# jhbastek/PhysicsInformedDiffusionModels

Measured on NVIDIA H100. Metric: train samples/s Darcy 64x64 PIDM, higher is better.
Workload: dtype bf16

## Files before the change

physicsinformeddiffusionmodels_b200/csrc/attention_fused.cu:

```cuda
#include "common.cuh"
#include "mma_util.cuh"
#include "pidm.h"

namespace pidm {

constexpr int LF_C = 32;

__device__ __forceinline__ uint32_t movm_t(uint32_t x) {
    uint32_t y;
    asm volatile("movmatrix.sync.aligned.m8n8.trans.b16 %0, %1;" : "=r"(y) : "r"(x));
    return y;
}

__device__ __forceinline__ void load_w_frags(uint32_t (&w)[2][4][2], const __nv_bfloat16* __restrict__ Wrows, int lane) {
    const int g = lane >> 2, t = lane & 3;
#pragma unroll
    for (int ks = 0; ks < 2; ++ks)
#pragma unroll
        for (int nt = 0; nt < 4; ++nt) {
            const uint32_t* row = reinterpret_cast<const uint32_t*>(Wrows + (size_t)(nt * 8 + g) * LF_C + ks * 16 + 2 * t);
            w[ks][nt][0] = __ldg(row);
            w[ks][nt][1] = __ldg(row + 4);
        }
}
template <int MT>
__device__ __forceinline__ void load_x_frags(uint32_t (&a)[MT][2][4], const __nv_bfloat16* Xs, int lane) {
#pragma unroll
    for (int mt = 0; mt < MT; ++mt)
#pragma unroll
        for (int ks = 0; ks < 2; ++ks) frag_a_rowmajor(a[mt][ks], Xs, LW_PITCH, mt * 16, ks * 16, lane);
}
template <int MT>
__device__ __forceinline__ void project(float (&c)[MT][4][4], const uint32_t (&a)[MT][2][4], const uint32_t (&w)[2][4][2]) {
#pragma unroll
    for (int mt = 0; mt < MT; ++mt)
#pragma unroll
        for (int nt = 0; nt < 4; ++nt) {
#pragma unroll
            for (int i = 0; i < 4; ++i) c[mt][nt][i] = 0.f;
#pragma unroll
            for (int ks = 0; ks < 2; ++ks) mma_bf16(c[mt][nt], a[mt][ks], w[ks][nt][0], w[ks][nt][1]);
        }
}
__device__ __forceinline__ void frag_softmax(float (&c)[4][4], float mul) {
#pragma unroll
    for (int half = 0; half < 2; ++half) {
        float mx = -INFINITY;
#pragma unroll
        for (int nt = 0; nt < 4; ++nt) mx = fmaxf(mx, fmaxf(c[nt][half * 2], c[nt][half * 2 + 1]));
        mx = fmaxf(mx, __shfl_xor_sync(0xffffffffu, mx, 1));
        mx = fmaxf(mx, __shfl_xor_sync(0xffffffffu, mx, 2));
        float s = 0.f;
#pragma unroll
        for (int nt = 0; nt < 4; ++nt) {
            c[nt][half * 2] = __expf(c[nt][half * 2] - mx);
            c[nt][half * 2 + 1] = __expf(c[nt][half * 2 + 1] - mx);
            s += c[nt][half * 2] + c[nt][half * 2 + 1];
        }
        s += __shfl_xor_sync(0xffffffffu, s, 1);
        s += __shfl_xor_sync(0xffffffffu, s, 2);
        const float inv = mul / s;
#pragma unroll
        for (int nt = 0; nt < 4; ++nt) { c[nt][half * 2] *= inv; c[nt][half * 2 + 1] *= inv; }
    }
}
__device__ __forceinline__ void c_to_a(uint32_t (&a)[2][4], const float (&c)[4][4]) {
#pragma unroll
    for (int ks = 0; ks < 2; ++ks) {
        a[ks][0] = pack_bf16(c[2 * ks][0], c[2 * ks][1]);
        a[ks][1] = pack_bf16(c[2 * ks][2], c[2 * ks][3]);
        a[ks][2] = pack_bf16(c[2 * ks + 1][0], c[2 * ks + 1][1]);
        a[ks][3] = pack_bf16(c[2 * ks + 1][2], c[2 * ks + 1][3]);
    }
}
__device__ __forceinline__ void load_cols(float (&v)[8], const float* __restrict__ src, int lane) {
    const int t = lane & 3;
#pragma unroll
    for (int nt = 0; nt < 4; ++nt) { v[nt * 2] = src[nt * 8 + 2 * t]; v[nt * 2 + 1] = src[nt * 8 + 2 * t + 1]; }
}

constexpr int LFS_STAGES = 2;
__global__ void __launch_bounds__(256) laf_kmax_kernel(const __nv_bfloat16* __restrict__ xn,
                                                       const __nv_bfloat16* __restrict__ W, float* __restrict__ part,
                                                       int N, int rows_per_chunk) {
    pdl_trigger();
    pdl_wait();
    extern __shared__ __align__(16) unsigned char raw[];
    const int b = blockIdx.y, chunk = blockIdx.x, lane = threadIdx.x & 31, h = threadIdx.x >> 5;
    __nv_bfloat16* ring = reinterpret_cast<__nv_bfloat16*>(raw) + (size_t)h * (LFS_STAGES * LW_TILE);
    const int n_begin = chunk * rows_per_chunk, n_end = min(N, n_begin + rows_per_chunk);
    const int n_tiles = (n_end - n_begin) / 32;
    const __nv_bfloat16* xsrc = xn + ((size_t)b * N + n_begin) * LF_C;
    auto issue = [&](int it) {
        if (it < n_tiles) lw_issue<32>(ring + (size_t)(it % LFS_STAGES) * LW_TILE, xsrc + (size_t)it * 32 * LF_C, LF_C, lane);
        cp_commit();
    };
#pragma unroll
    for (int s = 0; s < LFS_STAGES; ++s) issue(s);
    uint32_t wk[2][4][2];
    load_w_frags(wk, W + (size_t)(LM_HID + h * LM_D) * LF_C, lane);
    float m[8];
#pragma unroll
    for (int i = 0; i < 8; ++i) m[i] = -INFINITY;
    for (int it = 0; it < n_tiles; ++it) {
        cp_wait<LFS_STAGES - 1>();
        __syncwarp();
        uint32_t ax[2][2][4];
        load_x_frags<2>(ax, ring + (size_t)(it % LFS_STAGES) * LW_TILE, lane);
        __syncwarp();
        issue(it + LFS_STAGES);
        float ck[2][4][4];
        project<2>(ck, ax, wk);
#pragma unroll
        for (int nt = 0; nt < 4; ++nt)
#pragma unroll
            for (int j = 0; j < 2; ++j)
                m[nt * 2 + j] = fmaxf(fmaxf(m[nt * 2 + j], fmaxf(ck[0][nt][j], ck[0][nt][2 + j])),
                                      fmaxf(ck[1][nt][j], ck[1][nt][2 + j]));
    }
#pragma unroll
    for (int off = 4; off < 32; off <<= 1)
#pragma unroll
        for (int i = 0; i < 8; ++i) m[i] = fmaxf(m[i], __shfl_xor_sync(0xffffffffu, m[i], off));
    if (lane < 4) {
        float* o = part + ((size_t)b * gridDim.x + chunk) * LM_HID + h * LM_D;
#pragma unroll
        for (int nt = 0; nt < 4; ++nt)
#pragma unroll
            for (int j = 0; j < 2; ++j) o[nt * 8 + 2 * lane + j] = m[nt * 2 + j];
    }
}

__global__ void laf_finalize_kernel(float* __restrict__ ctx, float* __restrict__ kzinv, int n_rows) {
    pdl_trigger();
    pdl_wait();
    const int row = blockIdx.x * (blockDim.x / 32) + (threadIdx.x >> 5), lane = threadIdx.x & 31;
    if (row >= n_rows) return;
    const float zi = 1.f / kzinv[row];
    ctx[(size_t)row * LM_D + lane] *= zi;
    __syncwarp();
    if (lane == 0) kzinv[row] = zi;
}

constexpr int LFP_WO_TILE = LF_C * LW_PITCH;

__device__ __forceinline__ void lfp_dout_acc(float (&c)[4][4], const uint32_t (&ady)[2][4], const __nv_bfloat16* Wo, int lane) {
#pragma unroll
    for (int nt = 0; nt < 4; ++nt)
#pragma unroll
        for (int i = 0; i < 4; ++i) c[nt][i] = 0.f;
#pragma unroll
    for (int kc = 0; kc < 2; ++kc)
#pragma unroll
        for (int np = 0; np < 2; ++np) {
            uint32_t bw[4];
            frag_b_krows(bw, Wo, LW_PITCH, kc * 16, np * 16, lane);
            mma_bf16(c[2 * np], ady[kc], bw[0], bw[1]);
            mma_bf16(c[2 * np + 1], ady[kc], bw[2], bw[3]);
        }
}
__device__ __forceinline__ void lfp_dout(uint32_t (&ag)[2][4], const __nv_bfloat16* dyt, const __nv_bfloat16* Wo, int lane) {
    uint32_t ady[2][4];
    frag_a_rowmajor(ady[0], dyt, LW_PITCH, 0, 0, lane);
    frag_a_rowmajor(ady[1], dyt, LW_PITCH, 0, 16, lane);
    float c[4][4];
    lfp_dout_acc(c, ady, Wo, lane);
    c_to_a(ag, c);
}

template <int MODE>
struct LfcCfg {
    static constexpr int STAGES = MODE == 0 ? 4 : 2;
    static constexpr int STAGE_ELEMS = MODE == 0 ? LW_TILE : 2 * LW_TILE;
    static constexpr size_t SMEM_BASE = (size_t)LM_HEADS * STAGES * STAGE_ELEMS * 2 + (size_t)LM_HEADS * 2 * LM_D * 4;
    static constexpr size_t SMEM = SMEM_BASE + (MODE == 1 ? (size_t)LM_HEADS * LFP_WO_TILE * 2 : 0);
};
template <int MODE>
__global__ void __launch_bounds__(256, 2) laf_ctx_kernel(const __nv_bfloat16* __restrict__ xn, const __nv_bfloat16* __restrict__ W,
                                                      const __nv_bfloat16* __restrict__ dy, const float* __restrict__ part,
                                                      int n_stat_chunks, float* __restrict__ kmax, float* __restrict__ kzinv,
                                                      float* __restrict__ ctx, int N, int chunk_px, float scale,
                                                      const __nv_bfloat16* __restrict__ w_out) {
    pdl_trigger();
    pdl_wait();
    extern __shared__ __align__(16) unsigned char raw[];
    constexpr int LFC_STAGES = LfcCfg<MODE>::STAGES, LFC_STAGE_ELEMS = LfcCfg<MODE>::STAGE_ELEMS;
    const int b = blockIdx.y, chunk = blockIdx.x, lane = threadIdx.x & 31, h = threadIdx.x >> 5;
    __nv_bfloat16* ring = reinterpret_cast<__nv_bfloat16*>(raw) + (size_t)h * (LFC_STAGES * LFC_STAGE_ELEMS);
    float* sM = reinterpret_cast<float*>(raw + (size_t)LM_HEADS * LFC_STAGES * LFC_STAGE_ELEMS * 2) + h * 2 * LM_D;
    float* sZi = sM + LM_D;
    __nv_bfloat16* Wo = reinterpret_cast<__nv_bfloat16*>(raw + LfcCfg<MODE>::SMEM_BASE) + h * LFP_WO_TILE;
    const int n_begin = chunk * chunk_px, n_end = min(N, n_begin + chunk_px);
    const int n_tiles = (n_end - n_begin) / 32;
    const size_t pix0 = (size_t)b * N + n_begin;
    const __nv_bfloat16* xsrc = xn + pix0 * LF_C;
    const __nv_bfloat16* gsrc = (MODE == 1) ? dy + pix0 * LF_C : nullptr;
    if (MODE == 1) {
        lw_issue<32>(Wo, w_out + h * LM_D, LM_HID, lane);
        cp_commit();
    }
    auto issue = [&](int it) {
        if (it < n_tiles) {
            __nv_bfloat16* buf = ring + (size_t)(it % LFC_STAGES) * LFC_STAGE_ELEMS;
            lw_issue<32>(buf, xsrc + (size_t)it * 32 * LF_C, LF_C, lane);
            if (MODE == 1) lw_issue<32>(buf + LW_TILE, gsrc + (size_t)it * 32 * LF_C, LF_C, lane);
        }
        cp_commit();
    };
#pragma unroll
    for (int s = 0; s < LFC_STAGES; ++s) issue(s);
    uint32_t w0[2][4][2], w1[2][4][2];
    load_w_frags(w0, W + (size_t)((MODE == 0 ? LM_HID : 0) + h * LM_D) * LF_C, lane);
    if (MODE == 0) load_w_frags(w1, W + (size_t)(2 * LM_HID + h * LM_D) * LF_C, lane);
    float Mc[8];
    float zacc[8];
#pragma unroll
    for (int i = 0; i < 8; ++i) zacc[i] = 0.f;
    if (MODE == 0) {
        const int c = h * LM_D + lane;
        float M = -INFINITY;
        for (int i = 0; i < n_stat_chunks; ++i) M = fmaxf(M, part[((size_t)b * n_stat_chunks + i) * LM_HID + c]);
        sM[lane] = M;
        if (chunk == 0) kmax[(size_t)b * LM_HID + c] = M;
        __syncwarp();
        load_cols(Mc, sM, lane);
    }
    float acc[2][4][4];
#pragma unroll
    for (int i = 0; i < 2; ++i)
#pragma unroll
        for (int j = 0; j < 4; ++j)
#pragma unroll
            for (int k = 0; k < 4; ++k) acc[i][j][k] = 0.f;
    for (int it = 0; it < n_tiles; ++it) {
        cp_wait<LFC_STAGES - 1>();
        __syncwarp();
        const __nv_bfloat16* buf = ring + (size_t)(it % LFC_STAGES) * LFC_STAGE_ELEMS;
        uint32_t ax[2][2][4];
        load_x_frags<2>(ax, buf, lane);
        uint32_t bv[2][4][2];
        if (MODE == 1) {
#pragma unroll
            for (int mt = 0; mt < 2; ++mt) {
                uint32_t ady[2][4];
                frag_a_rowmajor(ady[0], buf + LW_TILE, LW_PITCH, mt * 16, 0, lane);
                frag_a_rowmajor(ady[1], buf + LW_TILE, LW_PITCH, mt * 16, 16, lane);
                float cd[4][4];
                lfp_dout_acc(cd, ady, Wo, lane);
#pragma unroll
                for (int nt = 0; nt < 4; ++nt) {
                    bv[mt][nt][0] = movm_t(pack_bf16(cd[nt][0], cd[nt][1]));
                    bv[mt][nt][1] = movm_t(pack_bf16(cd[nt][2], cd[nt][3]));
                }
            }
        }
        __syncwarp();
        issue(it + LFC_STAGES);
        float cw[2][4][4];
        project<2>(cw, ax, w0);
        if (MODE == 0) {
#pragma unroll
            for (int mt = 0; mt < 2; ++mt)
#pragma unroll
                for (int nt = 0; nt < 4; ++nt)
#pragma unroll
                    for (int i = 0; i < 4; ++i) {
                        cw[mt][nt][i] = __expf(cw[mt][nt][i] - Mc[nt * 2 + (i & 1)]);
                        zacc[nt * 2 + (i & 1)] += cw[mt][nt][i];
                    }
            float cv[2][4][4];
            project<2>(cv, ax, w1);
#pragma unroll
            for (int mt = 0; mt < 2; ++mt)
#pragma unroll
                for (int nt = 0; nt < 4; ++nt) {
                    bv[mt][nt][0] = movm_t(pack_bf16(cv[mt][nt][0], cv[mt][nt][1]));
                    bv[mt][nt][1] = movm_t(pack_bf16(cv[mt][nt][2], cv[mt][nt][3]));
                }
        } else {
            frag_softmax(cw[0], scale);
            frag_softmax(cw[1], scale);
        }
#pragma unroll
        for (int mt = 0; mt < 2; ++mt) {
#pragma unroll
            for (int md = 0; md < 2; ++md) {
                uint32_t a[4];
                a[0] = movm_t(pack_bf16(cw[mt][2 * md][0], cw[mt][2 * md][1]));
                a[1] = movm_t(pack_bf16(cw[mt][2 * md + 1][0], cw[mt][2 * md + 1][1]));
                a[2] = movm_t(pack_bf16(cw[mt][2 * md][2], cw[mt][2 * md][3]));
                a[3] = movm_t(pack_bf16(cw[mt][2 * md + 1][2], cw[mt][2 * md + 1][3]));
#pragma unroll
                for (int ne = 0; ne < 4; ++ne) mma_bf16(acc[md][ne], a, bv[mt][ne][0], bv[mt][ne][1]);
            }
        }
    }
    const int g = lane >> 2, t = lane & 3;
    if (MODE == 0) {
#pragma unroll
        for (int off = 4; off < 32; off <<= 1)
#pragma unroll
            for (int i = 0; i < 8; ++i) zacc[i] += __shfl_xor_sync(0xffffffffu, zacc[i], off);
        if (lane < 4) {
#pragma unroll
            for (int nt = 0; nt < 4; ++nt)
#pragma unroll
                for (int j = 0; j < 2; ++j)
                    atomicAdd(kzinv + (size_t)b * LM_HID + h * LM_D + nt * 8 + 2 * lane + j, zacc[nt * 2 + j]);
        }
    }
    float* cb = ctx + ((size_t)b * LM_HEADS + h) * LM_D * LM_D;
#pragma unroll
    for (int md = 0; md < 2; ++md)
#pragma unroll
        for (int half = 0; half < 2; ++half) {
            const int d = md * 16 + g + half * 8;
            const float f = (MODE == 0) ? 1.f / (float)N : 1.f;
#pragma unroll
            for (int ne = 0; ne < 4; ++ne) {
                const int e = ne * 8 + 2 * t;
                atomicAdd(cb + d * LM_D + e, acc[md][ne][half * 2] * f);
                atomicAdd(cb + d * LM_D + e + 1, acc[md][ne][half * 2 + 1] * f);
            }
        }
}

constexpr int LFO_STAGES = 3;
constexpr int LFO_R_PITCH = LF_C + 8;
constexpr size_t LAF_OUT_SMEM = (size_t)LFO_STAGES * LW_TILE * 2 + (size_t)LM_HEADS * LFP_WO_TILE * 2 +
                                (size_t)LM_HEADS * 32 * LFO_R_PITCH * 4;
__global__ void __launch_bounds__(256) laf_out_kernel(const __nv_bfloat16* __restrict__ xn, const __nv_bfloat16* __restrict__ W,
                                                      const float* __restrict__ ctx, __nv_bfloat16* __restrict__ y, int N,
                                                      int chunk_px, float scale, const __nv_bfloat16* __restrict__ w_out,
                                                      const float* __restrict__ b_out,
                                                      const __nv_bfloat16* __restrict__ residual) {
    pdl_trigger();
    pdl_wait();
    extern __shared__ __align__(16) unsigned char raw[];
    const int b = blockIdx.y, chunk = blockIdx.x, lane = threadIdx.x & 31, h = threadIdx.x >> 5;
    __nv_bfloat16* ring = reinterpret_cast<__nv_bfloat16*>(raw);
    __nv_bfloat16* Wo = ring + LFO_STAGES * LW_TILE + h * LFP_WO_TILE;
    float* R = reinterpret_cast<float*>(ring + LFO_STAGES * LW_TILE + LM_HEADS * LFP_WO_TILE);
    const int n_begin = chunk * chunk_px, n_end = min(N, n_begin + chunk_px);
    const int n_tiles = (n_end - n_begin) / 32;
    const size_t pix0 = (size_t)b * N + n_begin;
    const __nv_bfloat16* xsrc = xn + pix0 * LF_C;
    lw_issue<32>(Wo, w_out + h * LM_D, LM_HID, lane);
    cp_commit();
    auto issue = [&](int it) {
        if (it < n_tiles && h == 0)
            lw_issue<32>(ring + (size_t)(it % LFO_STAGES) * LW_TILE, xsrc + (size_t)it * 32 * LF_C, LF_C, lane);
        cp_commit();
    };
#pragma unroll
    for (int s = 0; s < LFO_STAGES - 1; ++s) issue(s);
    uint32_t wq[2][4][2];
    load_w_frags(wq, W + (size_t)(h * LM_D) * LF_C, lane);
    const float* ch = ctx + ((size_t)b * LM_HEADS + h) * LM_D * LM_D;
    uint32_t bf[2][4][2];
#pragma unroll
    for (int ks = 0; ks < 2; ++ks)
#pragma unroll
        for (int nt = 0; nt < 4; ++nt) frag_b_global<true>(bf[ks][nt], ch, ks * 16, nt * 8, lane);
    const int g = lane >> 2, t = lane & 3;
    const int rrow = threadIdx.x >> 4, rcol = (threadIdx.x & 15) * 2;
    const float2 bias = make_float2(b_out[rcol], b_out[rcol + 1]);
    float* Rw = R + h * 32 * LFO_R_PITCH;
    for (int it = 0; it < n_tiles; ++it) {
        uint32_t ax[2][2][4];
        cp_wait<LFO_STAGES - 2>();
        __syncthreads();
        issue(it + LFO_STAGES - 1);
        load_x_frags<2>(ax, ring + (size_t)(it % LFO_STAGES) * LW_TILE, lane);
        __nv_bfloat162 res[2];
#pragma unroll
        for (int rh = 0; rh < 2; ++rh)
            res[rh] = *reinterpret_cast<const __nv_bfloat162*>(residual + (pix0 + (size_t)it * 32 + rrow + rh * 16) * LF_C + rcol);
        float cq[2][4][4];
        project<2>(cq, ax, wq);
#pragma unroll
        for (int mt = 0; mt < 2; ++mt) {
            frag_softmax(cq[mt], scale);
            uint32_t a[2][4];
            c_to_a(a, cq[mt]);
            float c[4][4];
#pragma unroll
            for (int i = 0; i < 4; ++i)
#pragma unroll
                for (int k = 0; k < 4; ++k) c[i][k] = 0.f;
#pragma unroll
            for (int ks = 0; ks < 2; ++ks)
#pragma unroll
                for (int nt = 0; nt < 4; ++nt) mma_bf16(c[nt], a[ks], bf[ks][nt][0], bf[ks][nt][1]);
            c_to_a(a, c);
            float yh[4][4];
#pragma unroll
            for (int i = 0; i < 4; ++i)
#pragma unroll
                for (int k = 0; k < 4; ++k) yh[i][k] = 0.f;
#pragma unroll
            for (int ke = 0; ke < 2; ++ke)
#pragma unroll
                for (int np = 0; np < 2; ++np) {
                    uint32_t bw[4];
                    frag_b_nrows(bw, Wo, LW_PITCH, np * 16, ke * 16, lane);
                    mma_bf16(yh[2 * np], a[ke], bw[0], bw[1]);
                    mma_bf16(yh[2 * np + 1], a[ke], bw[2], bw[3]);
                }
#pragma unroll
            for (int nt = 0; nt < 4; ++nt)
#pragma unroll
                for (int half = 0; half < 2; ++half)
                    *reinterpret_cast<float2*>(Rw + (mt * 16 + g + half * 8) * LFO_R_PITCH + nt * 8 + 2 * t) =
                        make_float2(yh[nt][half * 2], yh[nt][half * 2 + 1]);
        }
        __syncthreads();
#pragma unroll
        for (int rh = 0; rh < 2; ++rh) {
            const int row = rrow + rh * 16;
            const size_t pix = pix0 + (size_t)it * 32 + row;
            const float2 x = __bfloat1622float2(res[rh]);
            float sx = x.x + bias.x, sy = x.y + bias.y;
#pragma unroll
            for (int w = 0; w < LM_HEADS; ++w) {
                const float2 v = *reinterpret_cast<const float2*>(R + (w * 32 + row) * LFO_R_PITCH + rcol);
                sx += v.x;
                sy += v.y;
            }
            *reinterpret_cast<uint32_t*>(y + pix * LF_C + rcol) = pack_bf16(sx, sy);
        }
    }
}

constexpr int LFB_ROWS = 16;
constexpr int LFB_STAGES = 4;
constexpr int LFB_TILE = LFB_ROWS * LW_PITCH;

struct LfbTile {
    uint32_t ax[1][2][4], ag[2][4];
};
__device__ __forceinline__ void lfb_dq(float (&dq)[4][4], const LfbTile& tl, const uint32_t (&wq)[2][4][2],
                                       const uint32_t (&bc)[2][4][2], float scale) {
    float c1[1][4][4], c2[4][4];
    project<1>(c1, tl.ax, wq);
    frag_softmax(c1[0], 1.f);
#pragma unroll
    for (int nt = 0; nt < 4; ++nt) {
#pragma unroll
        for (int i = 0; i < 4; ++i) c2[nt][i] = 0.f;
#pragma unroll
        for (int ks = 0; ks < 2; ++ks) mma_bf16(c2[nt], tl.ag[ks], bc[ks][nt][0], bc[ks][nt][1]);
    }
#pragma unroll
    for (int half = 0; half < 2; ++half) {
        float dot = 0.f;
#pragma unroll
        for (int nt = 0; nt < 4; ++nt)
            dot += c1[0][nt][half * 2] * c2[nt][half * 2] + c1[0][nt][half * 2 + 1] * c2[nt][half * 2 + 1];
        dot += __shfl_xor_sync(0xffffffffu, dot, 1);
        dot += __shfl_xor_sync(0xffffffffu, dot, 2);
#pragma unroll
        for (int nt = 0; nt < 4; ++nt)
#pragma unroll
            for (int j = 0; j < 2; ++j) dq[nt][half * 2 + j] = scale * c1[0][nt][half * 2 + j] * (c2[nt][half * 2 + j] - dot);
    }
}
__device__ __forceinline__ void lfb_dkdv(float (&dk)[4][4], float (&dv)[4][4], const uint32_t (&ax)[1][2][4],
                                         const uint32_t (&wk)[2][4][2], const uint32_t (&wv)[2][4][2],
                                         const uint32_t (&bd)[2][4][2], const uint32_t (&bt)[2][4][2],
                                         const float (&Mc)[8], const float (&Zc)[8], const float (&cdc)[8], float invN) {
    float c1[1][4][4];
    uint32_t a[2][4];
    project<1>(c1, ax, wv);
    c_to_a(a, c1[0]);
#pragma unroll
    for (int nt = 0; nt < 4; ++nt) {
#pragma unroll
        for (int i = 0; i < 4; ++i) dk[nt][i] = 0.f;
#pragma unroll
        for (int ks = 0; ks < 2; ++ks) mma_bf16(dk[nt], a[ks], bd[ks][nt][0], bd[ks][nt][1]);
    }
    project<1>(c1, ax, wk);
#pragma unroll
    for (int nt = 0; nt < 4; ++nt)
#pragma unroll
        for (int i = 0; i < 4; ++i) {
            c1[0][nt][i] = __expf(c1[0][nt][i] - Mc[nt * 2 + (i & 1)]) * Zc[nt * 2 + (i & 1)];
            dk[nt][i] = c1[0][nt][i] * (dk[nt][i] * invN - cdc[nt * 2 + (i & 1)]);
        }
    c_to_a(a, c1[0]);
#pragma unroll
    for (int nt = 0; nt < 4; ++nt) {
#pragma unroll
        for (int i = 0; i < 4; ++i) dv[nt][i] = 0.f;
#pragma unroll
        for (int ks = 0; ks < 2; ++ks) mma_bf16(dv[nt], a[ks], bt[ks][nt][0], bt[ks][nt][1]);
#pragma unroll
        for (int i = 0; i < 4; ++i) dv[nt][i] *= invN;
    }
}
__device__ __forceinline__ void lfb_cd(float (&cdc)[8], float* scd, const float* __restrict__ cg, const float* __restrict__ dg,
                                       int lane) {
    float s = 0.f;
#pragma unroll
    for (int e = 0; e < LM_D; e += 4) {
        const float4 x = *reinterpret_cast<const float4*>(dg + lane * LM_D + e);
        const float4 y = *reinterpret_cast<const float4*>(cg + lane * LM_D + e);
        s += x.x * y.x + x.y * y.y + x.z * y.z + x.w * y.w;
    }
    scd[lane] = s;
    __syncwarp();
    load_cols(cdc, scd, lane);
}

constexpr int LFB_W_PITCH = LF_C + 8;
constexpr int LFB_R_PITCH = LF_C + 8;
struct LfbCfg {
    static constexpr int STAGE_ELEMS = 2 * LFB_TILE;
    static constexpr size_t SMEM_BASE = (size_t)LFB_STAGES * STAGE_ELEMS * 2 + (size_t)3 * LM_HID * LFB_W_PITCH * 2 +
                                        (size_t)LM_HEADS * LFB_ROWS * LFB_R_PITCH * 4 + (size_t)LM_HEADS * LM_D * 4;
    static constexpr size_t SMEM = SMEM_BASE + (size_t)LM_HEADS * LFP_WO_TILE * 2;
};

__device__ __forceinline__ void mma_w(float (&c)[4][4], const uint32_t (&g)[2][4], const __nv_bfloat16* Wh, int lane) {
#pragma unroll
    for (int kd = 0; kd < 2; ++kd)
#pragma unroll
        for (int np = 0; np < 2; ++np) {
            uint32_t bw[4];
            frag_b_krows(bw, Wh, LFB_W_PITCH, kd * 16, np * 16, lane);
            mma_bf16(c[2 * np], g[kd], bw[0], bw[1]);
            mma_bf16(c[2 * np + 1], g[kd], bw[2], bw[3]);
        }
}

__global__ void __launch_bounds__(256) laf_bwd_kernel(const __nv_bfloat16* __restrict__ xn, const __nv_bfloat16* __restrict__ W,
                                                      const __nv_bfloat16* __restrict__ dy, const float* __restrict__ ctx,
                                                      const float* __restrict__ dctx, const float* __restrict__ kmax,
                                                      const float* __restrict__ kzinv, __nv_bfloat16* __restrict__ dxn,
                                                      int N, int chunk_px, float scale, const __nv_bfloat16* __restrict__ w_out) {
    pdl_trigger();
    pdl_wait();
    extern __shared__ __align__(16) unsigned char raw[];
    constexpr int LFB_STAGE_ELEMS = LfbCfg::STAGE_ELEMS;
    const int b = blockIdx.y, chunk = blockIdx.x, lane = threadIdx.x & 31, h = threadIdx.x >> 5;
    __nv_bfloat16* ring = reinterpret_cast<__nv_bfloat16*>(raw);
    __nv_bfloat16* Ws = ring + LFB_STAGES * LFB_STAGE_ELEMS;
    __nv_bfloat16* Wo = reinterpret_cast<__nv_bfloat16*>(raw + LfbCfg::SMEM_BASE) + h * LFP_WO_TILE;
    float* R = reinterpret_cast<float*>(Ws + 3 * LM_HID * LFB_W_PITCH);
    float* scd = R + LM_HEADS * LFB_ROWS * LFB_R_PITCH + h * LM_D;
    const int n_begin = chunk * chunk_px, n_end = min(N, n_begin + chunk_px);
    const int n_tiles = (n_end - n_begin) / LFB_ROWS;
    const size_t pix0 = (size_t)b * N + n_begin;
    const __nv_bfloat16* xsrc = xn + pix0 * LF_C;
    const __nv_bfloat16* gsrc = dy + pix0 * LF_C;
    for (int i = threadIdx.x; i < 3 * LM_HID * (LF_C / 8); i += blockDim.x)
        cp_async16(Ws + (i >> 2) * LFB_W_PITCH + (i & 3) * 8, W + (size_t)(i >> 2) * LF_C + (i & 3) * 8);
    lw_issue<32>(Wo, w_out + h * LM_D, LM_HID, lane);
    cp_commit();
    auto issue = [&](int it) {
        if (it < n_tiles) {
            __nv_bfloat16* buf = ring + (size_t)(it % LFB_STAGES) * LFB_STAGE_ELEMS;
            if (h == 0) lw_issue<LFB_ROWS>(buf, xsrc + (size_t)it * LFB_ROWS * LF_C, LF_C, lane);
            if (h == 1) lw_issue<LFB_ROWS>(buf + LFB_TILE, gsrc + (size_t)it * LFB_ROWS * LF_C, LF_C, lane);
        }
        cp_commit();
    };
#pragma unroll
    for (int s = 0; s < LFB_STAGES - 1; ++s) issue(s);
    const float* cg = ctx + ((size_t)b * LM_HEADS + h) * LM_D * LM_D;
    const float* dg = dctx + ((size_t)b * LM_HEADS + h) * LM_D * LM_D;
    float Mc[8], Zc[8], cdc[8];
    lfb_cd(cdc, scd, cg, dg, lane);
    load_cols(Mc, kmax + (size_t)b * LM_HID + h * LM_D, lane);
    load_cols(Zc, kzinv + (size_t)b * LM_HID + h * LM_D, lane);
    uint32_t wq[2][4][2], wk[2][4][2], wv[2][4][2];
    load_w_frags(wq, W + (size_t)(h * LM_D) * LF_C, lane);
    load_w_frags(wk, W + (size_t)(LM_HID + h * LM_D) * LF_C, lane);
    load_w_frags(wv, W + (size_t)(2 * LM_HID + h * LM_D) * LF_C, lane);
    uint32_t bc[2][4][2], bd[2][4][2], bt[2][4][2];
#pragma unroll
    for (int ks = 0; ks < 2; ++ks)
#pragma unroll
        for (int nt = 0; nt < 4; ++nt) {
            frag_b_global<false>(bc[ks][nt], cg, ks * 16, nt * 8, lane);
            frag_b_global<false>(bd[ks][nt], dg, ks * 16, nt * 8, lane);
            frag_b_global<true>(bt[ks][nt], dg, ks * 16, nt * 8, lane);
        }
    const int g = lane >> 2, t = lane & 3;
    const float invN = 1.f / (float)N;
    const __nv_bfloat16* Wq = Ws + (size_t)(h * LM_D) * LFB_W_PITCH;
    const __nv_bfloat16* Wk = Wq + (size_t)LM_HID * LFB_W_PITCH;
    const __nv_bfloat16* Wv = Wk + (size_t)LM_HID * LFB_W_PITCH;
    float* Rw = R + h * LFB_ROWS * LFB_R_PITCH;
    const int rrow = threadIdx.x >> 4, rcol = (threadIdx.x & 15) * 2;
    for (int it = 0; it < n_tiles; ++it) {
        cp_wait<LFB_STAGES - 2>();
        __syncthreads();
        issue(it + LFB_STAGES - 1);
        const __nv_bfloat16* buf = ring + (size_t)(it % LFB_STAGES) * LFB_STAGE_ELEMS;
        LfbTile tl;
        load_x_frags<1>(tl.ax, buf, lane);
        lfp_dout(tl.ag, buf + LFB_TILE, Wo, lane);
        float dx[4][4];
#pragma unroll
        for (int nt = 0; nt < 4; ++nt)
#pragma unroll
            for (int i = 0; i < 4; ++i) dx[nt][i] = 0.f;
        uint32_t a[2][4];
        {
            float dq[4][4];
            lfb_dq(dq, tl, wq, bc, scale);
            c_to_a(a, dq);
            mma_w(dx, a, Wq, lane);
        }
        {
            float dk[4][4], dv[4][4];
            lfb_dkdv(dk, dv, tl.ax, wk, wv, bd, bt, Mc, Zc, cdc, invN);
            c_to_a(a, dk);
            mma_w(dx, a, Wk, lane);
            c_to_a(a, dv);
            mma_w(dx, a, Wv, lane);
        }
#pragma unroll
        for (int nt = 0; nt < 4; ++nt)
#pragma unroll
            for (int half = 0; half < 2; ++half)
                *reinterpret_cast<float2*>(Rw + (g + half * 8) * LFB_R_PITCH + nt * 8 + 2 * t) =
                    make_float2(dx[nt][half * 2], dx[nt][half * 2 + 1]);
        __syncthreads();
        float sx = 0.f, sy = 0.f;
#pragma unroll
        for (int w = 0; w < LM_HEADS; ++w) {
            const float2 v = *reinterpret_cast<const float2*>(R + (w * LFB_ROWS + rrow) * LFB_R_PITCH + rcol);
            sx += v.x;
            sy += v.y;
        }
        *reinterpret_cast<uint32_t*>(dxn + (pix0 + (size_t)it * LFB_ROWS + rrow) * LF_C + rcol) = pack_bf16(sx, sy);
    }
}

template <int PART>
struct LfwCfg {
    static constexpr int STAGE_ELEMS = (PART == 0 ? 2 : 1) * LFB_TILE;
    static constexpr int S_PITCH = LM_D + 1;
    static_assert(LFB_STAGES * STAGE_ELEMS * 2 >= LM_D * S_PITCH * 4, "the epilogue staging reuses the tile ring");
    static constexpr size_t SMEM_BASE = (size_t)LM_HEADS * (LFB_STAGES * STAGE_ELEMS * 2 + LM_D * 4);
    static constexpr size_t SMEM = SMEM_BASE + (PART == 0 ? (size_t)LM_HEADS * LFP_WO_TILE * 2 : 0);
};

__device__ __forceinline__ void acc_gtx(float (&acc)[2][4][4], const float (&gf)[4][4], const uint32_t (&bx)[2][4]) {
#pragma unroll
    for (int md = 0; md < 2; ++md) {
        uint32_t a[4];
        a[0] = movm_t(pack_bf16(gf[2 * md][0], gf[2 * md][1]));
        a[1] = movm_t(pack_bf16(gf[2 * md + 1][0], gf[2 * md + 1][1]));
        a[2] = movm_t(pack_bf16(gf[2 * md][2], gf[2 * md][3]));
        a[3] = movm_t(pack_bf16(gf[2 * md + 1][2], gf[2 * md + 1][3]));
#pragma unroll
        for (int np = 0; np < 2; ++np) {
            mma_bf16(acc[md][2 * np], a, bx[np][0], bx[np][1]);
            mma_bf16(acc[md][2 * np + 1], a, bx[np][2], bx[np][3]);
        }
    }
}

template <int PART>
__global__ void __launch_bounds__(256) laf_wgrad_kernel(const __nv_bfloat16* __restrict__ xn, const __nv_bfloat16* __restrict__ W,
                                                        const __nv_bfloat16* __restrict__ dy, const float* __restrict__ ctx,
                                                        const float* __restrict__ dctx, const float* __restrict__ kmax,
                                                        const float* __restrict__ kzinv, float* __restrict__ grad_w, int N,
                                                        int chunk_px, long long w_stride_n, long long w_stride_c, float scale,
                                                        const __nv_bfloat16* __restrict__ w_out, float* __restrict__ grad_wo,
                                                        long long wo_stride_n, long long wo_stride_c) {
    pdl_trigger();
    pdl_wait();
    extern __shared__ __align__(16) unsigned char raw[];
    using Cfg = LfwCfg<PART>;
    constexpr int STAGE_ELEMS = Cfg::STAGE_ELEMS, S_PITCH = Cfg::S_PITCH;
    const int b = blockIdx.y, chunk = blockIdx.x, lane = threadIdx.x & 31, h = threadIdx.x >> 5;
    __nv_bfloat16* ring = reinterpret_cast<__nv_bfloat16*>(raw) + (size_t)h * (LFB_STAGES * STAGE_ELEMS);
    float* scd = reinterpret_cast<float*>(raw + (size_t)LM_HEADS * LFB_STAGES * STAGE_ELEMS * 2) + h * LM_D;
    __nv_bfloat16* Wo = reinterpret_cast<__nv_bfloat16*>(raw + Cfg::SMEM_BASE) + h * LFP_WO_TILE;
    const int n_begin = chunk * chunk_px, n_end = min(N, n_begin + chunk_px);
    const int n_tiles = (n_end - n_begin) / LFB_ROWS;
    const size_t pix0 = (size_t)b * N + n_begin;
    const __nv_bfloat16* xsrc = xn + pix0 * LF_C;
    const __nv_bfloat16* gsrc = dy + pix0 * LF_C;
    if (PART == 0) {
        lw_issue<32>(Wo, w_out + h * LM_D, LM_HID, lane);
        cp_commit();
    }
    auto issue = [&](int it) {
        if (it < n_tiles) {
            __nv_bfloat16* buf = ring + (size_t)(it % LFB_STAGES) * STAGE_ELEMS;
            lw_issue<LFB_ROWS>(buf, xsrc + (size_t)it * LFB_ROWS * LF_C, LF_C, lane);
            if (PART == 0) lw_issue<LFB_ROWS>(buf + LFB_TILE, gsrc + (size_t)it * LFB_ROWS * LF_C, LF_C, lane);
        }
        cp_commit();
    };
#pragma unroll
    for (int s = 0; s < LFB_STAGES; ++s) issue(s);
    const float* cg = ctx + ((size_t)b * LM_HEADS + h) * LM_D * LM_D;
    const float* dg = dctx + ((size_t)b * LM_HEADS + h) * LM_D * LM_D;
    float Mc[8], Zc[8], cdc[8];
    uint32_t w0[2][4][2], w1[2][4][2];
    uint32_t b0[2][4][2], b1[2][4][2];
    if (PART == 0) {
        load_w_frags(w0, W + (size_t)(h * LM_D) * LF_C, lane);
    } else {
        lfb_cd(cdc, scd, cg, dg, lane);
        load_cols(Mc, kmax + (size_t)b * LM_HID + h * LM_D, lane);
        load_cols(Zc, kzinv + (size_t)b * LM_HID + h * LM_D, lane);
        load_w_frags(w0, W + (size_t)(LM_HID + h * LM_D) * LF_C, lane);
        load_w_frags(w1, W + (size_t)(2 * LM_HID + h * LM_D) * LF_C, lane);
    }
#pragma unroll
    for (int ks = 0; ks < 2; ++ks)
#pragma unroll
        for (int nt = 0; nt < 4; ++nt) {
            frag_b_global<false>(b0[ks][nt], PART == 0 ? cg : dg, ks * 16, nt * 8, lane);
            frag_b_global<true>(b1[ks][nt], PART == 1 ? dg : cg, ks * 16, nt * 8, lane);
        }
    const float invN = 1.f / (float)N;
    float acc[2][2][4][4];
#pragma unroll
    for (int m = 0; m < 2; ++m)
#pragma unroll
        for (int i = 0; i < 2; ++i)
#pragma unroll
            for (int j = 0; j < 4; ++j)
#pragma unroll
                for (int k = 0; k < 4; ++k) acc[m][i][j][k] = 0.f;
    for (int it = 0; it < n_tiles; ++it) {
        cp_wait<LFB_STAGES - 1>();
        __syncwarp();
        const __nv_bfloat16* buf = ring + (size_t)(it % LFB_STAGES) * STAGE_ELEMS;
        LfbTile tl;
        load_x_frags<1>(tl.ax, buf, lane);
        uint32_t bx[2][4];
        frag_b_krows(bx[0], buf, LW_PITCH, 0, 0, lane);
        frag_b_krows(bx[1], buf, LW_PITCH, 0, 16, lane);
        uint32_t ady[2][4], bdy[2][4];
        if (PART == 0) {
            frag_a_rowmajor(ady[0], buf + LFB_TILE, LW_PITCH, 0, 0, lane);
            frag_a_rowmajor(ady[1], buf + LFB_TILE, LW_PITCH, 0, 16, lane);
            frag_b_krows(bdy[0], buf + LFB_TILE, LW_PITCH, 0, 0, lane);
            frag_b_krows(bdy[1], buf + LFB_TILE, LW_PITCH, 0, 16, lane);
        }
        __syncwarp();
        issue(it + LFB_STAGES);
        if (PART == 0) {
            {
                float c[4][4];
                lfp_dout_acc(c, ady, Wo, lane);
                c_to_a(tl.ag, c);
            }
            float dq[4][4];
            lfb_dq(dq, tl, w0, b0, scale);
            acc_gtx(acc[0], dq, bx);
            float cq[1][4][4], o[4][4];
            project<1>(cq, tl.ax, w0);
            frag_softmax(cq[0], scale);
            uint32_t a[2][4];
            c_to_a(a, cq[0]);
#pragma unroll
            for (int nt = 0; nt < 4; ++nt) {
#pragma unroll
                for (int i = 0; i < 4; ++i) o[nt][i] = 0.f;
#pragma unroll
                for (int ks = 0; ks < 2; ++ks) mma_bf16(o[nt], a[ks], b1[ks][nt][0], b1[ks][nt][1]);
            }
            acc_gtx(acc[1], o, bdy);
        } else {
            float dk[4][4], dv[4][4];
            lfb_dkdv(dk, dv, tl.ax, w0, w1, b0, b1, Mc, Zc, cdc, invN);
            acc_gtx(acc[0], dk, bx);
            acc_gtx(acc[1], dv, bx);
        }
    }
    cp_wait<0>();
    __syncwarp();
    float* S = reinterpret_cast<float*>(ring);
    const int g = lane >> 2, t = lane & 3;
#pragma unroll
    for (int m = 0; m < 2; ++m) {
#pragma unroll
        for (int md = 0; md < 2; ++md)
#pragma unroll
            for (int nc = 0; nc < 4; ++nc)
#pragma unroll
                for (int i = 0; i < 4; ++i) S[(md * 16 + g + 8 * (i >> 1)) * S_PITCH + nc * 8 + 2 * t + (i & 1)] = acc[m][md][nc][i];
        __syncwarp();
        if (PART == 0 && m == 1) {
            float* dst = grad_wo + (long long)(h * LM_D + lane) * wo_stride_c;
#pragma unroll 4
            for (int c = 0; c < LF_C; ++c) atomicAdd(dst + c * wo_stride_n, S[lane * S_PITCH + c]);
        } else {
            float* dst = grad_w + (long long)((PART + m) * LM_HID + h * LM_D) * w_stride_n + lane * w_stride_c;
#pragma unroll 4
            for (int d = 0; d < LM_D; ++d) atomicAdd(dst + d * w_stride_n, S[d * S_PITCH + lane]);
        }
        __syncwarp();
    }
}

constexpr size_t LAF_STATS_SMEM = (size_t)LM_HEADS * LFS_STAGES * LW_TILE * 2;

static int laf_attrs() {
    static bool done = false;
    if (!done) {
        PIDM_CUDA(cudaFuncSetAttribute(laf_kmax_kernel, cudaFuncAttributeMaxDynamicSharedMemorySize, (int)LAF_STATS_SMEM));
        PIDM_CUDA(cudaFuncSetAttribute(laf_ctx_kernel<0>, cudaFuncAttributeMaxDynamicSharedMemorySize, (int)LfcCfg<0>::SMEM));
        PIDM_CUDA(cudaFuncSetAttribute(laf_ctx_kernel<1>, cudaFuncAttributeMaxDynamicSharedMemorySize, (int)LfcCfg<1>::SMEM));
        PIDM_CUDA(cudaFuncSetAttribute(laf_out_kernel, cudaFuncAttributeMaxDynamicSharedMemorySize, (int)LAF_OUT_SMEM));
        PIDM_CUDA(cudaFuncSetAttribute(laf_bwd_kernel, cudaFuncAttributeMaxDynamicSharedMemorySize, (int)LfbCfg::SMEM));
        PIDM_CUDA(cudaFuncSetAttribute(laf_wgrad_kernel<0>, cudaFuncAttributeMaxDynamicSharedMemorySize, (int)LfwCfg<0>::SMEM));
        PIDM_CUDA(cudaFuncSetAttribute(laf_wgrad_kernel<1>, cudaFuncAttributeMaxDynamicSharedMemorySize, (int)LfwCfg<1>::SMEM));
        done = true;
    }
    return 0;
}

static int laf_chunk_px(int B, int N, int ctas_per_sm) {
    int k = (num_sms() * ctas_per_sm) / B;
    if (k < 1) k = 1;
    int px = ((N + k - 1) / k + 31) / 32 * 32;
    if (px < 64) px = 64;
    if (px > N) px = N;
    return px;
}
static int laf_stat_chunks(int N) {
    int c = N / 128;
    if (c < 1) c = 1;
    if (c > 16) c = 16;
    return c;
}

}
using namespace pidm;

extern "C" int pidm_linattn_block_supported(int C, int heads, int N, int dtype) {
    return (C == LF_C && heads == LM_HEADS && dtype == PIDM_BF16 && N % 128 == 0) ? 1 : 0;
}

extern "C" int pidm_linattn_block_workspace_floats(int B, int N) { return B * laf_stat_chunks(N) * LM_HID; }

extern "C" int pidm_linattn_block_plan(int B, int N, int* out) {
    PIDM_REQUIRE(N % 128 == 0 && B > 0, "linattn_block_plan: N must be a multiple of 128 (got %d)", N);
    const int v[5] = {laf_stat_chunks(N), laf_chunk_px(B, N, 2), laf_chunk_px(B, N, 2), laf_chunk_px(B, N, 1),
                      laf_chunk_px(B, N, 1)};
    for (int i = 0; i < 5; ++i) out[i] = v[i];
    return 0;
}

extern "C" int pidm_linattn_block_fwd(const void* xn, const void* w_qkv, const void* w_out, const float* b_out,
                                      const void* residual, void* y, float* ctx, float* kmax, float* kzinv,
                                      float* workspace, int B, int N, void* stream) {
    PIDM_REQUIRE(w_out && b_out && residual, "linattn_block_fwd: w_out, b_out and residual are required");
    PIDM_REQUIRE(N % 128 == 0, "linattn_block: N must be a multiple of 128 (got %d)", N);
    cudaStream_t st = (cudaStream_t)stream;
    if (int e = laf_attrs()) return e;
    const float scale = 0.17677669529663687f;
    const __nv_bfloat16* x = (const __nv_bfloat16*)xn;
    const __nv_bfloat16* w = (const __nv_bfloat16*)w_qkv;
    PIDM_CUDA(cudaMemsetAsync(ctx, 0, (size_t)B * LM_HEADS * LM_D * LM_D * sizeof(float), st));
    PIDM_CUDA(cudaMemsetAsync(kzinv, 0, (size_t)B * LM_HID * sizeof(float), st));
    const int chunks = laf_stat_chunks(N);
    const int rpc = N / chunks;
    PIDM_REQUIRE(rpc % 32 == 0 && rpc * chunks == N, "linattn_block: bad statistics chunking for N=%d", N);
    PIDM_CUDA(launch_plain(laf_kmax_kernel, dim3(dim3(chunks, B)), dim3(256), (size_t)(LAF_STATS_SMEM), st, x, w, workspace, N, rpc));
    const int px = laf_chunk_px(B, N, 2);
    const dim3 grid((N + px - 1) / px, B);
    PIDM_CUDA(launch_plain(laf_ctx_kernel<0>, grid, dim3(256), LfcCfg<0>::SMEM, st, x, w, nullptr, workspace, chunks, kmax, kzinv,
                           ctx, N, px, scale, nullptr));
    PIDM_CUDA(launch_plain(laf_finalize_kernel, dim3((B * LM_HID + 7) / 8), dim3(256), (size_t)(0), st, ctx, kzinv, B * LM_HID));
    PIDM_CUDA(launch_plain(laf_out_kernel, grid, dim3(256), LAF_OUT_SMEM, st, x, w, ctx, (__nv_bfloat16*)y, N, px, scale,
                           (const __nv_bfloat16*)w_out, b_out, (const __nv_bfloat16*)residual));
    PIDM_LAUNCH_CHECK("linattn_block_fwd");
    return 0;
}

extern "C" int pidm_linattn_block_bwd(const void* xn, const void* w_qkv, const void* w_out, const void* dy, const float* ctx,
                                      const float* kmax, const float* kzinv, void* dxn, float* dctx, int B, int N,
                                      void* stream) {
    PIDM_REQUIRE(N % 128 == 0, "linattn_block: N must be a multiple of 128 (got %d)", N);
    cudaStream_t st = (cudaStream_t)stream;
    if (int e = laf_attrs()) return e;
    const float scale = 0.17677669529663687f;
    const __nv_bfloat16* x = (const __nv_bfloat16*)xn;
    const __nv_bfloat16* w = (const __nv_bfloat16*)w_qkv;
    const __nv_bfloat16* wo = (const __nv_bfloat16*)w_out;
    const __nv_bfloat16* g = (const __nv_bfloat16*)dy;
    PIDM_CUDA(cudaMemsetAsync(dctx, 0, (size_t)B * LM_HEADS * LM_D * LM_D * sizeof(float), st));
    const int cpx = laf_chunk_px(B, N, 2);
    PIDM_CUDA(launch_plain(laf_ctx_kernel<1>, dim3(dim3((N + cpx - 1) / cpx, B)), dim3(256), LfcCfg<1>::SMEM, st, x, w, g,
                           nullptr, 0, nullptr, nullptr, dctx, N, cpx, scale, wo));
    const int bpx = laf_chunk_px(B, N, 1);
    PIDM_CUDA(launch_plain(laf_bwd_kernel, dim3(dim3((N + bpx - 1) / bpx, B)), dim3(256), LfbCfg::SMEM, st, x, w, g, ctx, dctx,
                           kmax, kzinv, (__nv_bfloat16*)dxn, N, bpx, scale, wo));
    PIDM_LAUNCH_CHECK("linattn_block_bwd");
    return 0;
}

extern "C" int pidm_linattn_block_wgrad(const void* xn, const void* w_qkv, const void* w_out, const void* dy,
                                        const float* ctx, const float* dctx, const float* kmax, const float* kzinv,
                                        float* grad_w_qkv, long long qkv_stride_n, long long qkv_stride_c,
                                        float* grad_w_out, long long out_stride_n, long long out_stride_c, int B, int N,
                                        void* stream) {
    PIDM_REQUIRE(N % 128 == 0, "linattn_block: N must be a multiple of 128 (got %d)", N);
    cudaStream_t st = (cudaStream_t)stream;
    if (int e = laf_attrs()) return e;
    const float scale = 0.17677669529663687f;
    const __nv_bfloat16* x = (const __nv_bfloat16*)xn;
    const __nv_bfloat16* w = (const __nv_bfloat16*)w_qkv;
    const __nv_bfloat16* wo = (const __nv_bfloat16*)w_out;
    const __nv_bfloat16* g = (const __nv_bfloat16*)dy;
    const int px = laf_chunk_px(B, N, 1);
    const dim3 grid((N + px - 1) / px, B);
    PIDM_CUDA(launch_plain(laf_wgrad_kernel<0>, grid, dim3(256), LfwCfg<0>::SMEM, st, x, w, g, ctx, dctx, kmax, kzinv, grad_w_qkv,
                           N, px, qkv_stride_n, qkv_stride_c, scale, wo, grad_w_out, out_stride_n, out_stride_c));
    PIDM_CUDA(launch_plain(laf_wgrad_kernel<1>, grid, dim3(256), LfwCfg<1>::SMEM, st, x, w, g, ctx, dctx, kmax, kzinv, grad_w_qkv,
                           N, px, qkv_stride_n, qkv_stride_c, scale, nullptr, nullptr, 0LL, 0LL));
    PIDM_LAUNCH_CHECK("linattn_block_wgrad");
    return 0;
}
```

physicsinformeddiffusionmodels_b200/csrc/hopper.cuh:

```cuda
#pragma once
#include "common.cuh"
#include <cuda.h>

namespace pidm {

__device__ __forceinline__ uint32_t smem_u32(const void* p) { return (uint32_t)__cvta_generic_to_shared(p); }

__device__ __forceinline__ void mbar_init(uint64_t* bar, int count) {
    asm volatile("mbarrier.init.shared::cta.b64 [%0], %1;" ::"r"(smem_u32(bar)), "r"(count));
}
__device__ __forceinline__ void mbar_expect_tx(uint64_t* bar, uint32_t bytes) {
    asm volatile("mbarrier.arrive.expect_tx.shared::cta.b64 _, [%0], %1;" ::"r"(smem_u32(bar)), "r"(bytes) : "memory");
}
__device__ __forceinline__ void mbar_arrive(uint64_t* bar) {
    asm volatile("mbarrier.arrive.shared::cta.b64 _, [%0];" ::"r"(smem_u32(bar)) : "memory");
}
__device__ __forceinline__ void mbar_wait(uint64_t* bar, uint32_t parity) {
    uint32_t ok;
    do {
        asm volatile(
            "{\n\t.reg .pred p;\n\t"
            "mbarrier.try_wait.parity.shared::cta.b64 p, [%1], %2;\n\t"
            "selp.u32 %0, 1, 0, p;\n\t}"
            : "=r"(ok)
            : "r"(smem_u32(bar)), "r"(parity)
            : "memory");
    } while (!ok);
}
__device__ __forceinline__ void tma_load_4d(void* dst, const CUtensorMap* map, uint64_t* bar, int c0, int c1, int c2,
                                            int c3) {
    asm volatile(
        "cp.async.bulk.tensor.4d.shared::cluster.global.mbarrier::complete_tx::bytes [%0], [%1, {%3, %4, %5, %6}], [%2];" ::"r"(
            smem_u32(dst)),
        "l"(map), "r"(smem_u32(bar)), "r"(c0), "r"(c1), "r"(c2), "r"(c3)
        : "memory");
}
__device__ __forceinline__ void tma_load_2d(void* dst, const CUtensorMap* map, uint64_t* bar, int c0, int c1) {
    asm volatile(
        "cp.async.bulk.tensor.2d.shared::cluster.global.mbarrier::complete_tx::bytes [%0], [%1, {%3, %4}], [%2];" ::"r"(
            smem_u32(dst)),
        "l"(map), "r"(smem_u32(bar)), "r"(c0), "r"(c1)
        : "memory");
}
__device__ __forceinline__ bool elect_one() {
    uint32_t pred;
    asm volatile(
        "{\n\t.reg .pred p;\n\t"
        "elect.sync _|p, 0xffffffff;\n\t"
        "selp.u32 %0, 1, 0, p;\n\t}"
        : "=r"(pred));
    return pred != 0;
}
__device__ __forceinline__ void named_bar(int id, int threads) {
    asm volatile("bar.sync %0, %1;" ::"r"(id), "r"(threads) : "memory");
}

template <int SWIZZLE_BYTES>
__host__ __device__ constexpr uint32_t gmma_desc_hi() {
    return (uint32_t)((8 * SWIZZLE_BYTES) >> 4) | ((SWIZZLE_BYTES == 128 ? 1u : 2u) << 30);
}
__device__ __forceinline__ uint32_t gmma_desc_lo(uint32_t smem_addr, uint32_t lbo_bytes) {
    return ((smem_addr & 0x3FFFF) >> 4) | (((lbo_bytes >> 4) & 0x3FFF) << 16);
}
__device__ __forceinline__ uint64_t gmma_desc(uint32_t hi, uint32_t lo) { return ((uint64_t)hi << 32) | lo; }

__device__ __forceinline__ void wgmma_fence() { asm volatile("wgmma.fence.sync.aligned;" ::: "memory"); }
__device__ __forceinline__ void wgmma_commit() { asm volatile("wgmma.commit_group.sync.aligned;" ::: "memory"); }
template <int PENDING>
__device__ __forceinline__ void wgmma_wait() { asm volatile("wgmma.wait_group.sync.aligned %0;" ::"n"(PENDING) : "memory"); }

template <int TRANS>
__device__ __forceinline__ void wgmma_bf16(float (&d)[16], uint64_t da, uint64_t db, uint32_t scale_d) {
    asm volatile(
        "{\n\t.reg .pred p;\n\t"
        "setp.ne.b32 p, %18, 0;\n\t"
        "wgmma.mma_async.sync.aligned.m64n32k16.f32.bf16.bf16 "
        "{%0, %1, %2, %3, %4, %5, %6, %7, %8, %9, %10, %11, %12, %13, %14, %15}, "
        "%16, %17, p, 1, 1, %19, %19;\n\t}"
        : "+f"(d[0]), "+f"(d[1]), "+f"(d[2]), "+f"(d[3]), "+f"(d[4]), "+f"(d[5]), "+f"(d[6]), "+f"(d[7]), "+f"(d[8]), "+f"(d[9]), "+f"(d[10]), "+f"(d[11]), "+f"(d[12]), "+f"(d[13]), "+f"(d[14]), "+f"(d[15])
        : "l"(da), "l"(db), "r"(scale_d), "n"(TRANS)
        : "memory");
}

template <int TRANS>
__device__ __forceinline__ void wgmma_bf16(float (&d)[32], uint64_t da, uint64_t db, uint32_t scale_d) {
    asm volatile(
        "{\n\t.reg .pred p;\n\t"
        "setp.ne.b32 p, %34, 0;\n\t"
        "wgmma.mma_async.sync.aligned.m64n64k16.f32.bf16.bf16 "
        "{%0, %1, %2, %3, %4, %5, %6, %7, %8, %9, %10, %11, %12, %13, %14, %15, %16, %17, %18, %19, %20, %21, %22, %23, %24, %25, %26, %27, %28, %29, %30, %31}, "
        "%32, %33, p, 1, 1, %35, %35;\n\t}"
        : "+f"(d[0]), "+f"(d[1]), "+f"(d[2]), "+f"(d[3]), "+f"(d[4]), "+f"(d[5]), "+f"(d[6]), "+f"(d[7]), "+f"(d[8]), "+f"(d[9]), "+f"(d[10]), "+f"(d[11]), "+f"(d[12]), "+f"(d[13]), "+f"(d[14]), "+f"(d[15]), "+f"(d[16]), "+f"(d[17]), "+f"(d[18]), "+f"(d[19]), "+f"(d[20]), "+f"(d[21]), "+f"(d[22]), "+f"(d[23]), "+f"(d[24]), "+f"(d[25]), "+f"(d[26]), "+f"(d[27]), "+f"(d[28]), "+f"(d[29]), "+f"(d[30]), "+f"(d[31])
        : "l"(da), "l"(db), "r"(scale_d), "n"(TRANS)
        : "memory");
}

template <int TRANS>
__device__ __forceinline__ void wgmma_bf16(float (&d)[64], uint64_t da, uint64_t db, uint32_t scale_d) {
    asm volatile(
        "{\n\t.reg .pred p;\n\t"
        "setp.ne.b32 p, %66, 0;\n\t"
        "wgmma.mma_async.sync.aligned.m64n128k16.f32.bf16.bf16 "
        "{%0, %1, %2, %3, %4, %5, %6, %7, %8, %9, %10, %11, %12, %13, %14, %15, %16, %17, %18, %19, %20, %21, %22, %23, %24, %25, %26, %27, %28, %29, %30, %31, %32, %33, %34, %35, %36, %37, %38, %39, %40, %41, %42, %43, %44, %45, %46, %47, %48, %49, %50, %51, %52, %53, %54, %55, %56, %57, %58, %59, %60, %61, %62, %63}, "
        "%64, %65, p, 1, 1, %67, %67;\n\t}"
        : "+f"(d[0]), "+f"(d[1]), "+f"(d[2]), "+f"(d[3]), "+f"(d[4]), "+f"(d[5]), "+f"(d[6]), "+f"(d[7]), "+f"(d[8]), "+f"(d[9]), "+f"(d[10]), "+f"(d[11]), "+f"(d[12]), "+f"(d[13]), "+f"(d[14]), "+f"(d[15]), "+f"(d[16]), "+f"(d[17]), "+f"(d[18]), "+f"(d[19]), "+f"(d[20]), "+f"(d[21]), "+f"(d[22]), "+f"(d[23]), "+f"(d[24]), "+f"(d[25]), "+f"(d[26]), "+f"(d[27]), "+f"(d[28]), "+f"(d[29]), "+f"(d[30]), "+f"(d[31]), "+f"(d[32]), "+f"(d[33]), "+f"(d[34]), "+f"(d[35]), "+f"(d[36]), "+f"(d[37]), "+f"(d[38]), "+f"(d[39]), "+f"(d[40]), "+f"(d[41]), "+f"(d[42]), "+f"(d[43]), "+f"(d[44]), "+f"(d[45]), "+f"(d[46]), "+f"(d[47]), "+f"(d[48]), "+f"(d[49]), "+f"(d[50]), "+f"(d[51]), "+f"(d[52]), "+f"(d[53]), "+f"(d[54]), "+f"(d[55]), "+f"(d[56]), "+f"(d[57]), "+f"(d[58]), "+f"(d[59]), "+f"(d[60]), "+f"(d[61]), "+f"(d[62]), "+f"(d[63])
        : "l"(da), "l"(db), "r"(scale_d), "n"(TRANS)
        : "memory");
}

typedef CUresult (*EncodeTiledFn)(CUtensorMap*, CUtensorMapDataType, cuuint32_t, void*, const cuuint64_t*,
                                  const cuuint64_t*, const cuuint32_t*, const cuuint32_t*, CUtensorMapInterleave,
                                  CUtensorMapSwizzle, CUtensorMapL2promotion, CUtensorMapFloatOOBfill);
EncodeTiledFn tensor_map_encoder();

}
```

Baseline: 7355.

## Port linear-attention kmax, output and backward kernels to Hopper wgmma

Rewrites the key-max statistics, fused output and backward kernels of the linear-attention block. They now use warpgroup wgmma on 64-row tiles staged in 64-byte-swizzled shared memory, replacing per-warp mma.sync on 32-row tiles. Weights and the bf16-converted context are held in shared memory once per CTA, and each warpgroup double-buffers its own tiles. The aim is to raise tensor-core throughput and cut fragment-loading overhead. In exchange it adds descriptor, fence and named-barrier complexity and uses coarser 64-pixel chunking, which may reduce the number of CTAs for small N.

```diff
diff --git a/physicsinformeddiffusionmodels_b200/csrc/attention_fused.cu b/physicsinformeddiffusionmodels_b200/csrc/attention_fused.cu
--- a/physicsinformeddiffusionmodels_b200/csrc/attention_fused.cu
+++ b/physicsinformeddiffusionmodels_b200/csrc/attention_fused.cu
@@ -1,4 +1,5 @@
 #include "common.cuh"
+#include "hopper.cuh"
 #include "mma_util.cuh"
 #include "pidm.h"
 
@@ -77,58 +78,6 @@
     const int t = lane & 3;
 #pragma unroll
     for (int nt = 0; nt < 4; ++nt) { v[nt * 2] = src[nt * 8 + 2 * t]; v[nt * 2 + 1] = src[nt * 8 + 2 * t + 1]; }
-}
-
-constexpr int LFS_STAGES = 2;
-__global__ void __launch_bounds__(256) laf_kmax_kernel(const __nv_bfloat16* __restrict__ xn,
-                                                       const __nv_bfloat16* __restrict__ W, float* __restrict__ part,
-                                                       int N, int rows_per_chunk) {
-    pdl_trigger();
-    pdl_wait();
-    extern __shared__ __align__(16) unsigned char raw[];
-    const int b = blockIdx.y, chunk = blockIdx.x, lane = threadIdx.x & 31, h = threadIdx.x >> 5;
-    __nv_bfloat16* ring = reinterpret_cast<__nv_bfloat16*>(raw) + (size_t)h * (LFS_STAGES * LW_TILE);
-    const int n_begin = chunk * rows_per_chunk, n_end = min(N, n_begin + rows_per_chunk);
-    const int n_tiles = (n_end - n_begin) / 32;
-    const __nv_bfloat16* xsrc = xn + ((size_t)b * N + n_begin) * LF_C;
-    auto issue = [&](int it) {
-        if (it < n_tiles) lw_issue<32>(ring + (size_t)(it % LFS_STAGES) * LW_TILE, xsrc + (size_t)it * 32 * LF_C, LF_C, lane);
-        cp_commit();
-    };
-#pragma unroll
-    for (int s = 0; s < LFS_STAGES; ++s) issue(s);
-    uint32_t wk[2][4][2];
-    load_w_frags(wk, W + (size_t)(LM_HID + h * LM_D) * LF_C, lane);
-    float m[8];
-#pragma unroll
-    for (int i = 0; i < 8; ++i) m[i] = -INFINITY;
-    for (int it = 0; it < n_tiles; ++it) {
-        cp_wait<LFS_STAGES - 1>();
-        __syncwarp();
-        uint32_t ax[2][2][4];
-        load_x_frags<2>(ax, ring + (size_t)(it % LFS_STAGES) * LW_TILE, lane);
-        __syncwarp();
-        issue(it + LFS_STAGES);
-        float ck[2][4][4];
-        project<2>(ck, ax, wk);
-#pragma unroll
-        for (int nt = 0; nt < 4; ++nt)
-#pragma unroll
-            for (int j = 0; j < 2; ++j)
-                m[nt * 2 + j] = fmaxf(fmaxf(m[nt * 2 + j], fmaxf(ck[0][nt][j], ck[0][nt][2 + j])),
-                                      fmaxf(ck[1][nt][j], ck[1][nt][2 + j]));
-    }
-#pragma unroll
-    for (int off = 4; off < 32; off <<= 1)
-#pragma unroll
-        for (int i = 0; i < 8; ++i) m[i] = fmaxf(m[i], __shfl_xor_sync(0xffffffffu, m[i], off));
-    if (lane < 4) {
-        float* o = part + ((size_t)b * gridDim.x + chunk) * LM_HID + h * LM_D;
-#pragma unroll
-        for (int nt = 0; nt < 4; ++nt)
-#pragma unroll
-            for (int j = 0; j < 2; ++j) o[nt * 8 + 2 * lane + j] = m[nt * 2 + j];
-    }
 }
 
 __global__ void laf_finalize_kernel(float* __restrict__ ctx, float* __restrict__ kzinv, int n_rows) {
@@ -159,15 +108,6 @@
             mma_bf16(c[2 * np + 1], ady[kc], bw[2], bw[3]);
         }
 }
-__device__ __forceinline__ void lfp_dout(uint32_t (&ag)[2][4], const __nv_bfloat16* dyt, const __nv_bfloat16* Wo, int lane) {
-    uint32_t ady[2][4];
-    frag_a_rowmajor(ady[0], dyt, LW_PITCH, 0, 0, lane);
-    frag_a_rowmajor(ady[1], dyt, LW_PITCH, 0, 16, lane);
-    float c[4][4];
-    lfp_dout_acc(c, ady, Wo, lane);
-    c_to_a(ag, c);
-}
-
 template <int MODE>
 struct LfcCfg {
     static constexpr int STAGES = MODE == 0 ? 4 : 2;
@@ -325,111 +265,223 @@
         }
 }
 
-constexpr int LFO_STAGES = 3;
-constexpr int LFO_R_PITCH = LF_C + 8;
-constexpr size_t LAF_OUT_SMEM = (size_t)LFO_STAGES * LW_TILE * 2 + (size_t)LM_HEADS * LFP_WO_TILE * 2 +
-                                (size_t)LM_HEADS * 32 * LFO_R_PITCH * 4;
-__global__ void __launch_bounds__(256) laf_out_kernel(const __nv_bfloat16* __restrict__ xn, const __nv_bfloat16* __restrict__ W,
-                                                      const float* __restrict__ ctx, __nv_bfloat16* __restrict__ y, int N,
-                                                      int chunk_px, float scale, const __nv_bfloat16* __restrict__ w_out,
-                                                      const float* __restrict__ b_out,
-                                                      const __nv_bfloat16* __restrict__ residual) {
+constexpr int LFO_WG = 2;
+constexpr int LFO_TILE_BYTES = 64 * LF_C * 2;
+constexpr int LFO_HEAD_BYTES = LM_D * LF_C * 2;
+constexpr size_t LFO_WQ = 0, LFO_WO = LFO_WQ + LM_HID * LF_C * 2, LFO_CTX = LFO_WO + LM_HEADS * LFO_HEAD_BYTES,
+                 LFO_RING = LFO_CTX + LM_HEADS * LFO_HEAD_BYTES;
+constexpr size_t LAF_OUT_SMEM = LFO_RING + (size_t)LFO_WG * 2 * LFO_TILE_BYTES + 1024;
+static_assert(LM_HID * 4 % (LFO_WG * 128) == 0, "the ctx gather loop has no tail");
+__device__ __forceinline__ uint32_t sw64(int r, int c) { return (uint32_t)(r * 64 + ((c ^ ((r >> 1) & 3)) << 4)); }
+
+__global__ void __launch_bounds__(LFO_WG * 128, 2) laf_out_kernel(const __nv_bfloat16* __restrict__ xn,
+                                                                 const __nv_bfloat16* __restrict__ W,
+                                                                 const float* __restrict__ ctx, __nv_bfloat16* __restrict__ y,
+                                                                 int N, int chunk_px, float scale,
+                                                                 const __nv_bfloat16* __restrict__ w_out,
+                                                                 const float* __restrict__ b_out,
+                                                                 const __nv_bfloat16* __restrict__ residual) {
     pdl_trigger();
     pdl_wait();
-    extern __shared__ __align__(16) unsigned char raw[];
-    const int b = blockIdx.y, chunk = blockIdx.x, lane = threadIdx.x & 31, h = threadIdx.x >> 5;
-    __nv_bfloat16* ring = reinterpret_cast<__nv_bfloat16*>(raw);
-    __nv_bfloat16* Wo = ring + LFO_STAGES * LW_TILE + h * LFP_WO_TILE;
-    float* R = reinterpret_cast<float*>(ring + LFO_STAGES * LW_TILE + LM_HEADS * LFP_WO_TILE);
+    extern __shared__ __align__(16) unsigned char raw_out[];
+    unsigned char* sm = reinterpret_cast<unsigned char*>((reinterpret_cast<uintptr_t>(raw_out) + 1023) & ~(uintptr_t)1023);
+    const int b = blockIdx.y, chunk = blockIdx.x, tid = threadIdx.x;
+    const int wg = tid >> 7, wt = tid & 127, warp = wt >> 5, lane = tid & 31, g = lane >> 2, t = lane & 3;
     const int n_begin = chunk * chunk_px, n_end = min(N, n_begin + chunk_px);
-    const int n_tiles = (n_end - n_begin) / 32;
+    const int n_tiles = (n_end - n_begin) / 64;
     const size_t pix0 = (size_t)b * N + n_begin;
-    const __nv_bfloat16* xsrc = xn + pix0 * LF_C;
-    lw_issue<32>(Wo, w_out + h * LM_D, LM_HID, lane);
-    cp_commit();
+    unsigned char* ring = sm + LFO_RING + (size_t)wg * 2 * LFO_TILE_BYTES;
     auto issue = [&](int it) {
-        if (it < n_tiles && h == 0)
-            lw_issue<32>(ring + (size_t)(it % LFO_STAGES) * LW_TILE, xsrc + (size_t)it * 32 * LF_C, LF_C, lane);
+        const int tile = wg + it * LFO_WG;
+        if (tile < n_tiles) {
+            unsigned char* dst = ring + (it & 1) * LFO_TILE_BYTES;
+            const __nv_bfloat16* src = xn + (pix0 + (size_t)tile * 64) * LF_C;
+#pragma unroll
+            for (int i = 0; i < 2; ++i) {
+                const int r = (wt >> 2) + 32 * i, c = wt & 3;
+                cp_async16(dst + sw64(r, c), src + r * LF_C + c * 8);
+            }
+        }
         cp_commit();
     };
-#pragma unroll
-    for (int s = 0; s < LFO_STAGES - 1; ++s) issue(s);
-    uint32_t wq[2][4][2];
-    load_w_frags(wq, W + (size_t)(h * LM_D) * LF_C, lane);
-    const float* ch = ctx + ((size_t)b * LM_HEADS + h) * LM_D * LM_D;
-    uint32_t bf[2][4][2];
-#pragma unroll
-    for (int ks = 0; ks < 2; ++ks)
-#pragma unroll
-        for (int nt = 0; nt < 4; ++nt) frag_b_global<true>(bf[ks][nt], ch, ks * 16, nt * 8, lane);
-    const int g = lane >> 2, t = lane & 3;
-    const int rrow = threadIdx.x >> 4, rcol = (threadIdx.x & 15) * 2;
-    const float2 bias = make_float2(b_out[rcol], b_out[rcol + 1]);
-    float* Rw = R + h * 32 * LFO_R_PITCH;
+    for (int i = tid; i < LM_HID * 4; i += LFO_WG * 128) {
+        const int r = i >> 2, c = i & 3;
+        cp_async16(sm + LFO_WQ + sw64(r, c), W + (size_t)r * LF_C + c * 8);
+        const int h = r >> 5, cc = r & 31;
+        cp_async16(sm + LFO_WO + h * LFO_HEAD_BYTES + sw64(cc, c), w_out + (size_t)cc * LM_HID + h * LM_D + c * 8);
+    }
+    cp_commit();
+    issue(0);
+    const float* cb = ctx + (size_t)b * LM_HEADS * LM_D * LM_D;
+#pragma unroll
+    for (int k = 0; k < LM_HID * 4 / (LFO_WG * 128); ++k) {
+        const int i = tid + k * LFO_WG * 128, r = i >> 2, c = i & 3, h = r >> 5, e = r & 31;
+        const float* src = cb + (size_t)h * LM_D * LM_D + (c * 8) * LM_D + e;
+        uint4 v;
+        v.x = pack_bf16(src[0 * LM_D], src[1 * LM_D]);
+        v.y = pack_bf16(src[2 * LM_D], src[3 * LM_D]);
+        v.z = pack_bf16(src[4 * LM_D], src[5 * LM_D]);
+        v.w = pack_bf16(src[6 * LM_D], src[7 * LM_D]);
+        *reinterpret_cast<uint4*>(sm + LFO_CTX + h * LFO_HEAD_BYTES + sw64(e, c)) = v;
+    }
+    float bias[8];
+#pragma unroll
+    for (int j = 0; j < 4; ++j) { bias[2 * j] = b_out[8 * j + 2 * t]; bias[2 * j + 1] = b_out[8 * j + 2 * t + 1]; }
+    cp_wait<1>();
+    fence_proxy_async();
+    __syncthreads();
+
+    constexpr uint32_t hi = gmma_desc_hi<64>();
+    const uint32_t wq_lo = gmma_desc_lo(smem_u32(sm + LFO_WQ), 16), wo_lo = gmma_desc_lo(smem_u32(sm + LFO_WO), 16),
+                   ctx_lo = gmma_desc_lo(smem_u32(sm + LFO_CTX), 16), ring_lo = gmma_desc_lo(smem_u32(ring), 16);
+    constexpr uint32_t head_lo = LFO_HEAD_BYTES >> 4, tile_lo = LFO_TILE_BYTES >> 4;
+    const int row0 = 16 * warp + g;
+    for (int it = 0; wg + it * LFO_WG < n_tiles; ++it) {
+        const size_t pix = pix0 + (size_t)(wg + it * LFO_WG) * 64;
+        uint32_t res[2][4];
+#pragma unroll
+        for (int half = 0; half < 2; ++half)
+#pragma unroll
+            for (int j = 0; j < 4; ++j)
+                res[half][j] = *reinterpret_cast<const uint32_t*>(residual + (pix + row0 + 8 * half) * LF_C + 8 * j + 2 * t);
+        cp_wait<0>();
+        fence_proxy_async();
+        named_bar(1 + wg, 128);
+        issue(it + 1);
+        const uint32_t x_lo = ring_lo + (it & 1) * tile_lo;
+        float acc[16];
+#pragma unroll
+        for (int hp = 0; hp < LM_HEADS / 2; ++hp) {
+            float q[2][4][4];
+            float(&qf)[32] = *reinterpret_cast<float(*)[32]>(&q[0][0][0]);
+            wgmma_fence();
+#pragma unroll
+            for (int ks = 0; ks < 2; ++ks)
+                wgmma_bf16<0>(qf, gmma_desc(hi, x_lo + 2 * ks), gmma_desc(hi, wq_lo + 2 * head_lo * hp + 2 * ks), ks);
+            wgmma_commit();
+            wgmma_wait<0>();
+            uint32_t a[2][2][4];
+#pragma unroll
+            for (int hh = 0; hh < 2; ++hh) {
+                frag_softmax(q[hh], scale);
+                c_to_a(a[hh], q[hh]);
+            }
+            float o[2][16];
+            wgmma_fence();
+#pragma unroll
+            for (int hh = 0; hh < 2; ++hh)
+#pragma unroll
+                for (int ks = 0; ks < 2; ++ks)
+                    wgmma_bf16_rs(o[hh], a[hh][ks], gmma_desc(hi, ctx_lo + head_lo * (2 * hp + hh) + 2 * ks), ks);
+            wgmma_commit();
+            wgmma_wait<0>();
+            uint32_t ao[2][2][4];
+#pragma unroll
+            for (int hh = 0; hh < 2; ++hh) c_to_a(ao[hh], *reinterpret_cast<const float(*)[4][4]>(&o[hh][0]));
+            wgmma_fence();
+#pragma unroll
+            for (int hh = 0; hh < 2; ++hh)
+#pragma unroll
+                for (int ks = 0; ks < 2; ++ks)
+                    wgmma_bf16_rs(acc, ao[hh][ks], gmma_desc(hi, wo_lo + head_lo * (2 * hp + hh) + 2 * ks),
+                                  (hp | hh | ks) != 0);
+            wgmma_commit();
+        }
+        wgmma_wait<0>();
+#pragma unroll
+        for (int half = 0; half < 2; ++half)
+#pragma unroll
+            for (int j = 0; j < 4; ++j) {
+                const float2 x = __bfloat1622float2(*reinterpret_cast<const __nv_bfloat162*>(&res[half][j]));
+                *reinterpret_cast<uint32_t*>(y + (pix + row0 + 8 * half) * LF_C + 8 * j + 2 * t) =
+                    pack_bf16(x.x + bias[2 * j] + acc[4 * j + 2 * half], x.y + bias[2 * j + 1] + acc[4 * j + 2 * half + 1]);
+            }
+    }
+}
+
+constexpr size_t LFS_WK = 0, LFS_RING = LM_HID * LF_C * 2;
+constexpr size_t LAF_STATS_SMEM = LFS_RING + 2 * LFO_TILE_BYTES + 1024;
+__global__ void __launch_bounds__(128) laf_kmax_kernel(const __nv_bfloat16* __restrict__ xn,
+                                                       const __nv_bfloat16* __restrict__ W, float* __restrict__ part,
+                                                       int N, int rows_per_chunk) {
+    pdl_trigger();
+    pdl_wait();
+    extern __shared__ __align__(16) unsigned char raw_kmax[];
+    unsigned char* sm = reinterpret_cast<unsigned char*>((reinterpret_cast<uintptr_t>(raw_kmax) + 1023) & ~(uintptr_t)1023);
+    const int b = blockIdx.y, chunk = blockIdx.x, tid = threadIdx.x, warp = tid >> 5, lane = tid & 31, t = lane & 3;
+    const int n_begin = chunk * rows_per_chunk, rows = min(N, n_begin + rows_per_chunk) - n_begin;
+    const int n_tiles = (rows + 63) / 64;
+    const __nv_bfloat16* src = xn + ((size_t)b * N + n_begin) * LF_C;
+    auto issue = [&](int it) {
+        if (it < n_tiles) {
+            unsigned char* dst = sm + LFS_RING + (it & 1) * LFO_TILE_BYTES;
+#pragma unroll
+            for (int i = 0; i < 2; ++i) {
+                const int r = (tid >> 2) + 32 * i, c = tid & 3;
+                if (it * 64 + r < rows) cp_async16(dst + sw64(r, c), src + (size_t)(it * 64 + r) * LF_C + c * 8);
+            }
+        }
+        cp_commit();
+    };
+    for (int i = tid; i < LM_HID * 4; i += 128)
+        cp_async16(sm + LFS_WK + sw64(i >> 2, i & 3), W + (size_t)(LM_HID + (i >> 2)) * LF_C + (i & 3) * 8);
+    cp_commit();
+    issue(0);
+    constexpr uint32_t hi = gmma_desc_hi<64>();
+    constexpr uint32_t pair_lo = 2 * LFO_HEAD_BYTES >> 4, tile_lo = LFO_TILE_BYTES >> 4;
+    const uint32_t wk_lo = gmma_desc_lo(smem_u32(sm + LFS_WK), 16), ring_lo = gmma_desc_lo(smem_u32(sm + LFS_RING), 16);
+    const int row0 = 16 * warp + (lane >> 2);
+    float m[LM_HEADS / 2][16];
+#pragma unroll
+    for (int hp = 0; hp < LM_HEADS / 2; ++hp)
+#pragma unroll
+        for (int i = 0; i < 16; ++i) m[hp][i] = -INFINITY;
     for (int it = 0; it < n_tiles; ++it) {
-        uint32_t ax[2][2][4];
-        cp_wait<LFO_STAGES - 2>();
+        cp_wait<0>();
+        fence_proxy_async();
         __syncthreads();
-        issue(it + LFO_STAGES - 1);
-        load_x_frags<2>(ax, ring + (size_t)(it % LFO_STAGES) * LW_TILE, lane);
-        __nv_bfloat162 res[2];
-#pragma unroll
-        for (int rh = 0; rh < 2; ++rh)
-            res[rh] = *reinterpret_cast<const __nv_bfloat162*>(residual + (pix0 + (size_t)it * 32 + rrow + rh * 16) * LF_C + rcol);
-        float cq[2][4][4];
-        project<2>(cq, ax, wq);
-#pragma unroll
-        for (int mt = 0; mt < 2; ++mt) {
-            frag_softmax(cq[mt], scale);
-            uint32_t a[2][4];
-            c_to_a(a, cq[mt]);
-            float c[4][4];
-#pragma unroll
-            for (int i = 0; i < 4; ++i)
-#pragma unroll
-                for (int k = 0; k < 4; ++k) c[i][k] = 0.f;
+        issue(it + 1);
+        const bool ok0 = it * 64 + row0 < rows, ok1 = it * 64 + row0 + 8 < rows;
+        const uint32_t x_lo = ring_lo + (it & 1) * tile_lo;
+#pragma unroll
+        for (int hp = 0; hp < LM_HEADS / 2; ++hp) {
+            float k[32];
+            wgmma_fence();
 #pragma unroll
             for (int ks = 0; ks < 2; ++ks)
-#pragma unroll
-                for (int nt = 0; nt < 4; ++nt) mma_bf16(c[nt], a[ks], bf[ks][nt][0], bf[ks][nt][1]);
-            c_to_a(a, c);
-            float yh[4][4];
-#pragma unroll
-            for (int i = 0; i < 4; ++i)
-#pragma unroll
-                for (int k = 0; k < 4; ++k) yh[i][k] = 0.f;
-#pragma unroll
-            for (int ke = 0; ke < 2; ++ke)
-#pragma unroll
-                for (int np = 0; np < 2; ++np) {
-                    uint32_t bw[4];
-                    frag_b_nrows(bw, Wo, LW_PITCH, np * 16, ke * 16, lane);
-                    mma_bf16(yh[2 * np], a[ke], bw[0], bw[1]);
-                    mma_bf16(yh[2 * np + 1], a[ke], bw[2], bw[3]);
+                wgmma_bf16<0>(k, gmma_desc(hi, x_lo + 2 * ks), gmma_desc(hi, wk_lo + pair_lo * hp + 2 * ks), ks);
+            wgmma_commit();
+            wgmma_wait<0>();
+#pragma unroll
+            for (int j = 0; j < 8; ++j)
+#pragma unroll
+                for (int jj = 0; jj < 2; ++jj) {
+                    if (ok0) m[hp][2 * j + jj] = fmaxf(m[hp][2 * j + jj], k[4 * j + jj]);
+                    if (ok1) m[hp][2 * j + jj] = fmaxf(m[hp][2 * j + jj], k[4 * j + 2 + jj]);
                 }
-#pragma unroll
-            for (int nt = 0; nt < 4; ++nt)
-#pragma unroll
-                for (int half = 0; half < 2; ++half)
-                    *reinterpret_cast<float2*>(Rw + (mt * 16 + g + half * 8) * LFO_R_PITCH + nt * 8 + 2 * t) =
-                        make_float2(yh[nt][half * 2], yh[nt][half * 2 + 1]);
-        }
-        __syncthreads();
-#pragma unroll
-        for (int rh = 0; rh < 2; ++rh) {
-            const int row = rrow + rh * 16;
-            const size_t pix = pix0 + (size_t)it * 32 + row;
-            const float2 x = __bfloat1622float2(res[rh]);
-            float sx = x.x + bias.x, sy = x.y + bias.y;
-#pragma unroll
-            for (int w = 0; w < LM_HEADS; ++w) {
-                const float2 v = *reinterpret_cast<const float2*>(R + (w * 32 + row) * LFO_R_PITCH + rcol);
-                sx += v.x;
-                sy += v.y;
-            }
-            *reinterpret_cast<uint32_t*>(y + pix * LF_C + rcol) = pack_bf16(sx, sy);
-        }
-    }
+        }
+    }
+#pragma unroll
+    for (int off = 4; off < 32; off <<= 1)
+#pragma unroll
+        for (int hp = 0; hp < LM_HEADS / 2; ++hp)
+#pragma unroll
+            for (int i = 0; i < 16; ++i) m[hp][i] = fmaxf(m[hp][i], __shfl_xor_sync(0xffffffffu, m[hp][i], off));
+    cp_wait<0>();
+    __syncthreads();
+    float* red = reinterpret_cast<float*>(sm + LFS_RING);
+    if (lane < 4) {
+#pragma unroll
+        for (int hp = 0; hp < LM_HEADS / 2; ++hp)
+#pragma unroll
+            for (int j = 0; j < 8; ++j)
+#pragma unroll
+                for (int jj = 0; jj < 2; ++jj) red[warp * LM_HID + hp * 64 + 8 * j + 2 * t + jj] = m[hp][2 * j + jj];
+    }
+    __syncthreads();
+    float* o = part + ((size_t)b * gridDim.x + chunk) * LM_HID;
+    for (int c = tid; c < LM_HID; c += 128)
+        o[c] = fmaxf(fmaxf(red[c], red[LM_HID + c]), fmaxf(red[2 * LM_HID + c], red[3 * LM_HID + c]));
 }
 
 constexpr int LFB_ROWS = 16;
@@ -513,130 +565,243 @@
     load_cols(cdc, scd, lane);
 }
 
-constexpr int LFB_W_PITCH = LF_C + 8;
-constexpr int LFB_R_PITCH = LF_C + 8;
-struct LfbCfg {
-    static constexpr int STAGE_ELEMS = 2 * LFB_TILE;
-    static constexpr size_t SMEM_BASE = (size_t)LFB_STAGES * STAGE_ELEMS * 2 + (size_t)3 * LM_HID * LFB_W_PITCH * 2 +
-                                        (size_t)LM_HEADS * LFB_ROWS * LFB_R_PITCH * 4 + (size_t)LM_HEADS * LM_D * 4;
-    static constexpr size_t SMEM = SMEM_BASE + (size_t)LM_HEADS * LFP_WO_TILE * 2;
-};
-
-__device__ __forceinline__ void mma_w(float (&c)[4][4], const uint32_t (&g)[2][4], const __nv_bfloat16* Wh, int lane) {
-#pragma unroll
-    for (int kd = 0; kd < 2; ++kd)
-#pragma unroll
-        for (int np = 0; np < 2; ++np) {
-            uint32_t bw[4];
-            frag_b_krows(bw, Wh, LFB_W_PITCH, kd * 16, np * 16, lane);
-            mma_bf16(c[2 * np], g[kd], bw[0], bw[1]);
-            mma_bf16(c[2 * np + 1], g[kd], bw[2], bw[3]);
-        }
-}
-
-__global__ void __launch_bounds__(256) laf_bwd_kernel(const __nv_bfloat16* __restrict__ xn, const __nv_bfloat16* __restrict__ W,
-                                                      const __nv_bfloat16* __restrict__ dy, const float* __restrict__ ctx,
-                                                      const float* __restrict__ dctx, const float* __restrict__ kmax,
-                                                      const float* __restrict__ kzinv, __nv_bfloat16* __restrict__ dxn,
-                                                      int N, int chunk_px, float scale, const __nv_bfloat16* __restrict__ w_out) {
+constexpr int LFB_WG = 3;
+constexpr int LFB_STAGE_BYTES = 2 * LFO_TILE_BYTES;
+constexpr size_t LFB_W = 0, LFB_WT = LFB_W + 3 * LM_HID * LF_C * 2, LFB_WOT = LFB_WT + 3 * LM_HID * LF_C * 2,
+                 LFB_CTX = LFB_WOT + LM_HEADS * LFO_HEAD_BYTES, LFB_DCTX = LFB_CTX + LM_HEADS * LFO_HEAD_BYTES,
+                 LFB_DCTXT = LFB_DCTX + LM_HEADS * LFO_HEAD_BYTES, LFB_STATS = LFB_DCTXT + LM_HEADS * LFO_HEAD_BYTES,
+                 LFB_RING = LFB_STATS + 4096;
+constexpr size_t LAF_BWD_SMEM = LFB_RING + (size_t)LFB_WG * 2 * LFB_STAGE_BYTES + 1024;
+static_assert(LAF_BWD_SMEM <= 227 * 1024, "one CTA per SM");
+static_assert(3 * LM_HID * 4 % (LFB_WG * 128) == 0, "the W^T gather loop has no tail");
+
+__device__ __forceinline__ void st_col8(unsigned char* tile, int r0, int col, uint4 v) {
+    const uint32_t w[4] = {v.x, v.y, v.z, v.w};
+#pragma unroll
+    for (int j = 0; j < 8; ++j)
+        *reinterpret_cast<uint16_t*>(tile + sw64(r0 + j, col >> 3) + (col & 7) * 2) = (uint16_t)(w[j >> 1] >> (16 * (j & 1)));
+}
+__device__ __forceinline__ uint4 ld8_bf16(const float* __restrict__ src) {
+    const float4 a = *reinterpret_cast<const float4*>(src), b = *reinterpret_cast<const float4*>(src + 4);
+    return make_uint4(pack_bf16(a.x, a.y), pack_bf16(a.z, a.w), pack_bf16(b.x, b.y), pack_bf16(b.z, b.w));
+}
+__device__ __forceinline__ float (&as_frag(float* p))[4][4] { return *reinterpret_cast<float(*)[4][4]>(p); }
+
+__global__ void __launch_bounds__(LFB_WG * 128, 1) laf_bwd_kernel(const __nv_bfloat16* __restrict__ xn,
+                                                                 const __nv_bfloat16* __restrict__ W,
+                                                                 const __nv_bfloat16* __restrict__ dy,
+                                                                 const float* __restrict__ ctx, const float* __restrict__ dctx,
+                                                                 const float* __restrict__ kmax,
+                                                                 const float* __restrict__ kzinv, __nv_bfloat16* __restrict__ dxn,
+                                                                 int N, int chunk_px, float scale,
+                                                                 const __nv_bfloat16* __restrict__ w_out) {
     pdl_trigger();
     pdl_wait();
-    extern __shared__ __align__(16) unsigned char raw[];
-    constexpr int LFB_STAGE_ELEMS = LfbCfg::STAGE_ELEMS;
-    const int b = blockIdx.y, chunk = blockIdx.x, lane = threadIdx.x & 31, h = threadIdx.x >> 5;
-    __nv_bfloat16* ring = reinterpret_cast<__nv_bfloat16*>(raw);
-    __nv_bfloat16* Ws = ring + LFB_STAGES * LFB_STAGE_ELEMS;
-    __nv_bfloat16* Wo = reinterpret_cast<__nv_bfloat16*>(raw + LfbCfg::SMEM_BASE) + h * LFP_WO_TILE;
-    float* R = reinterpret_cast<float*>(Ws + 3 * LM_HID * LFB_W_PITCH);
-    float* scd = R + LM_HEADS * LFB_ROWS * LFB_R_PITCH + h * LM_D;
+    extern __shared__ __align__(16) unsigned char raw_bwd[];
+    unsigned char* sm = reinterpret_cast<unsigned char*>((reinterpret_cast<uintptr_t>(raw_bwd) + 1023) & ~(uintptr_t)1023);
+    constexpr int NT = LFB_WG * 128;
+    const int b = blockIdx.y, chunk = blockIdx.x, tid = threadIdx.x;
+    const int wg = tid >> 7, wt = tid & 127, warp = wt >> 5, lane = tid & 31, t = lane & 3;
     const int n_begin = chunk * chunk_px, n_end = min(N, n_begin + chunk_px);
-    const int n_tiles = (n_end - n_begin) / LFB_ROWS;
+    const int n_tiles = (n_end - n_begin) / 64;
     const size_t pix0 = (size_t)b * N + n_begin;
-    const __nv_bfloat16* xsrc = xn + pix0 * LF_C;
-    const __nv_bfloat16* gsrc = dy + pix0 * LF_C;
-    for (int i = threadIdx.x; i < 3 * LM_HID * (LF_C / 8); i += blockDim.x)
-        cp_async16(Ws + (i >> 2) * LFB_W_PITCH + (i & 3) * 8, W + (size_t)(i >> 2) * LF_C + (i & 3) * 8);
-    lw_issue<32>(Wo, w_out + h * LM_D, LM_HID, lane);
-    cp_commit();
+    unsigned char* ring = sm + LFB_RING + (size_t)wg * 2 * LFB_STAGE_BYTES;
     auto issue = [&](int it) {
-        if (it < n_tiles) {
-            __nv_bfloat16* buf = ring + (size_t)(it % LFB_STAGES) * LFB_STAGE_ELEMS;
-            if (h == 0) lw_issue<LFB_ROWS>(buf, xsrc + (size_t)it * LFB_ROWS * LF_C, LF_C, lane);
-            if (h == 1) lw_issue<LFB_ROWS>(buf + LFB_TILE, gsrc + (size_t)it * LFB_ROWS * LF_C, LF_C, lane);
+        const int tile = wg + it * LFB_WG;
+        if (tile < n_tiles) {
+            unsigned char* dst = ring + (it & 1) * LFB_STAGE_BYTES;
+            const size_t off = (pix0 + (size_t)tile * 64) * LF_C;
+#pragma unroll
+            for (int i = 0; i < 2; ++i) {
+                const int r = (wt >> 2) + 32 * i, c = wt & 3;
+                cp_async16(dst + sw64(r, c), xn + off + r * LF_C + c * 8);
+                cp_async16(dst + LFO_TILE_BYTES + sw64(r, c), dy + off + r * LF_C + c * 8);
+            }
         }
         cp_commit();
     };
-#pragma unroll
-    for (int s = 0; s < LFB_STAGES - 1; ++s) issue(s);
-    const float* cg = ctx + ((size_t)b * LM_HEADS + h) * LM_D * LM_D;
-    const float* dg = dctx + ((size_t)b * LM_HEADS + h) * LM_D * LM_D;
-    float Mc[8], Zc[8], cdc[8];
-    lfb_cd(cdc, scd, cg, dg, lane);
-    load_cols(Mc, kmax + (size_t)b * LM_HID + h * LM_D, lane);
-    load_cols(Zc, kzinv + (size_t)b * LM_HID + h * LM_D, lane);
-    uint32_t wq[2][4][2], wk[2][4][2], wv[2][4][2];
-    load_w_frags(wq, W + (size_t)(h * LM_D) * LF_C, lane);
-    load_w_frags(wk, W + (size_t)(LM_HID + h * LM_D) * LF_C, lane);
-    load_w_frags(wv, W + (size_t)(2 * LM_HID + h * LM_D) * LF_C, lane);
-    uint32_t bc[2][4][2], bd[2][4][2], bt[2][4][2];
-#pragma unroll
-    for (int ks = 0; ks < 2; ++ks)
-#pragma unroll
-        for (int nt = 0; nt < 4; ++nt) {
-            frag_b_global<false>(bc[ks][nt], cg, ks * 16, nt * 8, lane);
-            frag_b_global<false>(bd[ks][nt], dg, ks * 16, nt * 8, lane);
-            frag_b_global<true>(bt[ks][nt], dg, ks * 16, nt * 8, lane);
-        }
-    const int g = lane >> 2, t = lane & 3;
+    for (int i = tid; i < 3 * LM_HID * 4; i += NT)
+        cp_async16(sm + LFB_W + sw64(i >> 2, i & 3), W + (size_t)(i >> 2) * LF_C + (i & 3) * 8);
+    cp_commit();
+    issue(0);
+    const float* cg = ctx + (size_t)b * LM_HEADS * LM_D * LM_D;
+    const float* dg = dctx + (size_t)b * LM_HEADS * LM_D * LM_D;
+#pragma unroll
+    for (int k = 0; k < 3 * LM_HID * 4 / NT; ++k) {
+        const int i = tid + k * NT, n = i >> 2, q = i & 3;
+        st_col8(sm + LFB_WT + (n >> 5) * LFO_HEAD_BYTES, q * 8, n & 31,
+                *reinterpret_cast<const uint4*>(W + (size_t)n * LF_C + q * 8));
+    }
+#pragma unroll
+    for (int k = 0; k < (LM_HID * 4 + NT - 1) / NT; ++k) {
+        const int i = tid + k * NT;
+        if (i >= LM_HID * 4) break;
+        {
+            const int c = i >> 5, q = i & 31;
+            st_col8(sm + LFB_WOT + (q >> 2) * LFO_HEAD_BYTES, (q & 3) * 8, c,
+                    *reinterpret_cast<const uint4*>(w_out + (size_t)c * LM_HID + q * 8));
+        }
+        const int r = i >> 2, q = i & 3, h = r >> 5, d = r & 31;
+        *reinterpret_cast<uint4*>(sm + LFB_CTX + h * LFO_HEAD_BYTES + sw64(d, q)) = ld8_bf16(cg + (size_t)r * LM_D + q * 8);
+        const uint4 v = ld8_bf16(dg + (size_t)r * LM_D + q * 8);
+        *reinterpret_cast<uint4*>(sm + LFB_DCTX + h * LFO_HEAD_BYTES + sw64(d, q)) = v;
+        st_col8(sm + LFB_DCTXT + h * LFO_HEAD_BYTES, q * 8, d, v);
+    }
+    float* sK = reinterpret_cast<float*>(sm + LFB_STATS);
+    float* sZ = sK + LM_HID;
+    float* sCD = sZ + LM_HID;
+    for (int r = tid; r < LM_HID; r += NT) {
+        sK[r] = kmax[(size_t)b * LM_HID + r];
+        sZ[r] = kzinv[(size_t)b * LM_HID + r];
+        float s = 0.f;
+#pragma unroll
+        for (int e = 0; e < LM_D; e += 4) {
+            const float4 x = *reinterpret_cast<const float4*>(dg + (size_t)r * LM_D + e);
+            const float4 y = *reinterpret_cast<const float4*>(cg + (size_t)r * LM_D + e);
+            s += x.x * y.x + x.y * y.y + x.z * y.z + x.w * y.w;
+        }
+        sCD[r] = s;
+    }
+    cp_wait<1>();
+    fence_proxy_async();
+    __syncthreads();
+
+    constexpr uint32_t hi = gmma_desc_hi<64>();
+    constexpr uint32_t head_lo = LFO_HEAD_BYTES >> 4, tile_lo = LFO_TILE_BYTES >> 4;
+    const uint32_t w_lo = gmma_desc_lo(smem_u32(sm + LFB_W), 16), wt_lo = gmma_desc_lo(smem_u32(sm + LFB_WT), 16),
+                   wot_lo = gmma_desc_lo(smem_u32(sm + LFB_WOT), 16), ctx_lo = gmma_desc_lo(smem_u32(sm + LFB_CTX), 16),
+                   dctx_lo = gmma_desc_lo(smem_u32(sm + LFB_DCTX), 16),
+                   dctxt_lo = gmma_desc_lo(smem_u32(sm + LFB_DCTXT), 16), ring_lo = gmma_desc_lo(smem_u32(ring), 16);
     const float invN = 1.f / (float)N;
-    const __nv_bfloat16* Wq = Ws + (size_t)(h * LM_D) * LFB_W_PITCH;
-    const __nv_bfloat16* Wk = Wq + (size_t)LM_HID * LFB_W_PITCH;
-    const __nv_bfloat16* Wv = Wk + (size_t)LM_HID * LFB_W_PITCH;
-    float* Rw = R + h * LFB_ROWS * LFB_R_PITCH;
-    const int rrow = threadIdx.x >> 4, rcol = (threadIdx.x & 15) * 2;
-    for (int it = 0; it < n_tiles; ++it) {
-        cp_wait<LFB_STAGES - 2>();
-        __syncthreads();
-        issue(it + LFB_STAGES - 1);
-        const __nv_bfloat16* buf = ring + (size_t)(it % LFB_STAGES) * LFB_STAGE_ELEMS;
-        LfbTile tl;
-        load_x_frags<1>(tl.ax, buf, lane);
-        lfp_dout(tl.ag, buf + LFB_TILE, Wo, lane);
-        float dx[4][4];
-#pragma unroll
-        for (int nt = 0; nt < 4; ++nt)
-#pragma unroll
-            for (int i = 0; i < 4; ++i) dx[nt][i] = 0.f;
-        uint32_t a[2][4];
-        {
-            float dq[4][4];
-            lfb_dq(dq, tl, wq, bc, scale);
-            c_to_a(a, dq);
-            mma_w(dx, a, Wq, lane);
-        }
-        {
-            float dk[4][4], dv[4][4];
-            lfb_dkdv(dk, dv, tl.ax, wk, wv, bd, bt, Mc, Zc, cdc, invN);
-            c_to_a(a, dk);
-            mma_w(dx, a, Wk, lane);
-            c_to_a(a, dv);
-            mma_w(dx, a, Wv, lane);
-        }
-#pragma unroll
-        for (int nt = 0; nt < 4; ++nt)
-#pragma unroll
-            for (int half = 0; half < 2; ++half)
-                *reinterpret_cast<float2*>(Rw + (g + half * 8) * LFB_R_PITCH + nt * 8 + 2 * t) =
-                    make_float2(dx[nt][half * 2], dx[nt][half * 2 + 1]);
-        __syncthreads();
-        float sx = 0.f, sy = 0.f;
-#pragma unroll
-        for (int w = 0; w < LM_HEADS; ++w) {
-            const float2 v = *reinterpret_cast<const float2*>(R + (w * LFB_ROWS + rrow) * LFB_R_PITCH + rcol);
-            sx += v.x;
-            sy += v.y;
-        }
-        *reinterpret_cast<uint32_t*>(dxn + (pix0 + (size_t)it * LFB_ROWS + rrow) * LF_C + rcol) = pack_bf16(sx, sy);
+    const int row0 = 16 * warp + (lane >> 2);
+    for (int it = 0; wg + it * LFB_WG < n_tiles; ++it) {
+        const size_t pix = pix0 + (size_t)(wg + it * LFB_WG) * 64;
+        cp_wait<0>();
+        fence_proxy_async();
+        named_bar(1 + wg, 128);
+        issue(it + 1);
+        const uint32_t x_lo = ring_lo + (it & 1) * 2 * tile_lo, y_lo = x_lo + tile_lo;
+        float dx[16];
+#pragma unroll 1
+        for (int hp = 0; hp < LM_HEADS / 2; ++hp) {
+            float qf[32], gf[32];
+            wgmma_fence();
+#pragma unroll
+            for (int ks = 0; ks < 2; ++ks) {
+                wgmma_bf16<0>(gf, gmma_desc(hi, y_lo + 2 * ks), gmma_desc(hi, wot_lo + head_lo * 2 * hp + 2 * ks), ks);
+                wgmma_bf16<0>(qf, gmma_desc(hi, x_lo + 2 * ks), gmma_desc(hi, w_lo + head_lo * 2 * hp + 2 * ks), ks);
+            }
+            wgmma_commit();
+            wgmma_wait<0>();
+            uint32_t ag[2][2][4];
+#pragma unroll
+            for (int hh = 0; hh < 2; ++hh) {
+                c_to_a(ag[hh], as_frag(gf + 16 * hh));
+                frag_softmax(as_frag(qf + 16 * hh), 1.f);
+            }
+            float dp[2][16], vf[32];
+            wgmma_fence();
+#pragma unroll
+            for (int ks = 0; ks < 2; ++ks) {
+#pragma unroll
+                for (int hh = 0; hh < 2; ++hh)
+                    wgmma_bf16_rs(dp[hh], ag[hh][ks], gmma_desc(hi, ctx_lo + head_lo * (2 * hp + hh) + 2 * ks), ks);
+                wgmma_bf16<0>(vf, gmma_desc(hi, x_lo + 2 * ks), gmma_desc(hi, w_lo + head_lo * (16 + 2 * hp) + 2 * ks), ks);
+            }
+            wgmma_commit();
+            wgmma_wait<0>();
+            uint32_t aq[2][2][4], av[2][2][4];
+#pragma unroll
+            for (int hh = 0; hh < 2; ++hh) {
+                float(&p)[4][4] = as_frag(qf + 16 * hh);
+                float(&d)[4][4] = as_frag(dp[hh]);
+#pragma unroll
+                for (int half = 0; half < 2; ++half) {
+                    float dot = 0.f;
+#pragma unroll
+                    for (int nt = 0; nt < 4; ++nt)
+                        dot += p[nt][half * 2] * d[nt][half * 2] + p[nt][half * 2 + 1] * d[nt][half * 2 + 1];
+                    dot += __shfl_xor_sync(0xffffffffu, dot, 1);
+                    dot += __shfl_xor_sync(0xffffffffu, dot, 2);
+#pragma unroll
+                    for (int nt = 0; nt < 4; ++nt)
+#pragma unroll
+                        for (int j = 0; j < 2; ++j) d[nt][half * 2 + j] = scale * p[nt][half * 2 + j] * (d[nt][half * 2 + j] - dot);
+                }
+                c_to_a(aq[hh], d);
+                c_to_a(av[hh], as_frag(vf + 16 * hh));
+            }
+            float dk[2][16], kf[32];
+            wgmma_fence();
+#pragma unroll
+            for (int ks = 0; ks < 2; ++ks) {
+#pragma unroll
+                for (int hh = 0; hh < 2; ++hh)
+                    wgmma_bf16_rs(dk[hh], av[hh][ks], gmma_desc(hi, dctx_lo + head_lo * (2 * hp + hh) + 2 * ks), ks);
+                wgmma_bf16<0>(kf, gmma_desc(hi, x_lo + 2 * ks), gmma_desc(hi, w_lo + head_lo * (8 + 2 * hp) + 2 * ks), ks);
+            }
+#pragma unroll
+            for (int hh = 0; hh < 2; ++hh)
+#pragma unroll
+                for (int ks = 0; ks < 2; ++ks)
+                    wgmma_bf16_rs(dx, aq[hh][ks], gmma_desc(hi, wt_lo + head_lo * (2 * hp + hh) + 2 * ks), (hp | hh | ks) != 0);
+            wgmma_commit();
+            wgmma_wait<0>();
+            uint32_t ak[2][2][4], adk[2][2][4];
+#pragma unroll
+            for (int hh = 0; hh < 2; ++hh) {
+                float(&k)[4][4] = as_frag(kf + 16 * hh);
+                float(&d)[4][4] = as_frag(dk[hh]);
+                const int col0 = (2 * hp + hh) * LM_D + 2 * t;
+#pragma unroll
+                for (int nt = 0; nt < 4; ++nt)
+#pragma unroll
+                    for (int j = 0; j < 2; ++j) {
+                        const int col = col0 + nt * 8 + j;
+                        const float M = sK[col], Z = sZ[col], cd = sCD[col];
+#pragma unroll
+                        for (int half = 0; half < 2; ++half) {
+                            const float kt = __expf(k[nt][half * 2 + j] - M) * Z;
+                            k[nt][half * 2 + j] = kt;
+                            d[nt][half * 2 + j] = kt * (d[nt][half * 2 + j] * invN - cd);
+                        }
+                    }
+                c_to_a(ak[hh], k);
+                c_to_a(adk[hh], d);
+            }
+            float dv[2][16];
+            wgmma_fence();
+#pragma unroll
+            for (int hh = 0; hh < 2; ++hh)
+#pragma unroll
+                for (int ks = 0; ks < 2; ++ks) {
+                    wgmma_bf16_rs(dv[hh], ak[hh][ks], gmma_desc(hi, dctxt_lo + head_lo * (2 * hp + hh) + 2 * ks), ks);
+                    wgmma_bf16_rs(dx, adk[hh][ks], gmma_desc(hi, wt_lo + head_lo * (8 + 2 * hp + hh) + 2 * ks), 1);
+                }
+            wgmma_commit();
+            wgmma_wait<0>();
+            uint32_t adv[2][2][4];
+#pragma unroll
+            for (int hh = 0; hh < 2; ++hh) {
+#pragma unroll
+                for (int i = 0; i < 16; ++i) dv[hh][i] *= invN;
+                c_to_a(adv[hh], as_frag(dv[hh]));
+            }
+            wgmma_fence();
+#pragma unroll
+            for (int hh = 0; hh < 2; ++hh)
+#pragma unroll
+                for (int ks = 0; ks < 2; ++ks)
+                    wgmma_bf16_rs(dx, adv[hh][ks], gmma_desc(hi, wt_lo + head_lo * (16 + 2 * hp + hh) + 2 * ks), 1);
+            wgmma_commit();
+        }
+        wgmma_wait<0>();
+#pragma unroll
+        for (int half = 0; half < 2; ++half)
+#pragma unroll
+            for (int j = 0; j < 4; ++j)
+                *reinterpret_cast<uint32_t*>(dxn + (pix + row0 + 8 * half) * LF_C + 8 * j + 2 * t) =
+                    pack_bf16(dx[4 * j + 2 * half], dx[4 * j + 2 * half + 1]);
     }
 }
 
@@ -805,7 +970,6 @@
     }
 }
 
-constexpr size_t LAF_STATS_SMEM = (size_t)LM_HEADS * LFS_STAGES * LW_TILE * 2;
 
 static int laf_attrs() {
     static bool done = false;
@@ -814,7 +978,7 @@
         PIDM_CUDA(cudaFuncSetAttribute(laf_ctx_kernel<0>, cudaFuncAttributeMaxDynamicSharedMemorySize, (int)LfcCfg<0>::SMEM));
         PIDM_CUDA(cudaFuncSetAttribute(laf_ctx_kernel<1>, cudaFuncAttributeMaxDynamicSharedMemorySize, (int)LfcCfg<1>::SMEM));
         PIDM_CUDA(cudaFuncSetAttribute(laf_out_kernel, cudaFuncAttributeMaxDynamicSharedMemorySize, (int)LAF_OUT_SMEM));
-        PIDM_CUDA(cudaFuncSetAttribute(laf_bwd_kernel, cudaFuncAttributeMaxDynamicSharedMemorySize, (int)LfbCfg::SMEM));
+        PIDM_CUDA(cudaFuncSetAttribute(laf_bwd_kernel, cudaFuncAttributeMaxDynamicSharedMemorySize, (int)LAF_BWD_SMEM));
         PIDM_CUDA(cudaFuncSetAttribute(laf_wgrad_kernel<0>, cudaFuncAttributeMaxDynamicSharedMemorySize, (int)LfwCfg<0>::SMEM));
         PIDM_CUDA(cudaFuncSetAttribute(laf_wgrad_kernel<1>, cudaFuncAttributeMaxDynamicSharedMemorySize, (int)LfwCfg<1>::SMEM));
         done = true;
@@ -822,10 +986,10 @@
     return 0;
 }
 
-static int laf_chunk_px(int B, int N, int ctas_per_sm) {
+static int laf_chunk_px(int B, int N, int ctas_per_sm, int granule = 32) {
     int k = (num_sms() * ctas_per_sm) / B;
     if (k < 1) k = 1;
-    int px = ((N + k - 1) / k + 31) / 32 * 32;
+    int px = ((N + k - 1) / k + granule - 1) / granule * granule;
     if (px < 64) px = 64;
     if (px > N) px = N;
     return px;
@@ -848,7 +1012,7 @@
 
 extern "C" int pidm_linattn_block_plan(int B, int N, int* out) {
     PIDM_REQUIRE(N % 128 == 0 && B > 0, "linattn_block_plan: N must be a multiple of 128 (got %d)", N);
-    const int v[5] = {laf_stat_chunks(N), laf_chunk_px(B, N, 2), laf_chunk_px(B, N, 2), laf_chunk_px(B, N, 1),
+    const int v[5] = {laf_stat_chunks(N), laf_chunk_px(B, N, 2), laf_chunk_px(B, N, 2, 64), laf_chunk_px(B, N, 1, 64),
                       laf_chunk_px(B, N, 1)};
     for (int i = 0; i < 5; ++i) out[i] = v[i];
     return 0;
@@ -869,13 +1033,14 @@
     const int chunks = laf_stat_chunks(N);
     const int rpc = N / chunks;
     PIDM_REQUIRE(rpc % 32 == 0 && rpc * chunks == N, "linattn_block: bad statistics chunking for N=%d", N);
-    PIDM_CUDA(launch_plain(laf_kmax_kernel, dim3(dim3(chunks, B)), dim3(256), (size_t)(LAF_STATS_SMEM), st, x, w, workspace, N, rpc));
+    PIDM_CUDA(launch_plain(laf_kmax_kernel, dim3(dim3(chunks, B)), dim3(128), LAF_STATS_SMEM, st, x, w, workspace, N, rpc));
     const int px = laf_chunk_px(B, N, 2);
-    const dim3 grid((N + px - 1) / px, B);
-    PIDM_CUDA(launch_plain(laf_ctx_kernel<0>, grid, dim3(256), LfcCfg<0>::SMEM, st, x, w, nullptr, workspace, chunks, kmax, kzinv,
-                           ctx, N, px, scale, nullptr));
+    PIDM_CUDA(launch_plain(laf_ctx_kernel<0>, dim3((N + px - 1) / px, B), dim3(256), LfcCfg<0>::SMEM, st, x, w, nullptr,
+                           workspace, chunks, kmax, kzinv, ctx, N, px, scale, nullptr));
     PIDM_CUDA(launch_plain(laf_finalize_kernel, dim3((B * LM_HID + 7) / 8), dim3(256), (size_t)(0), st, ctx, kzinv, B * LM_HID));
-    PIDM_CUDA(launch_plain(laf_out_kernel, grid, dim3(256), LAF_OUT_SMEM, st, x, w, ctx, (__nv_bfloat16*)y, N, px, scale,
+    const int opx = laf_chunk_px(B, N, 2, 64);
+    PIDM_CUDA(launch_plain(laf_out_kernel, dim3((N + opx - 1) / opx, B), dim3(LFO_WG * 128), LAF_OUT_SMEM, st, x, w, ctx,
+                           (__nv_bfloat16*)y, N, opx, scale,
                            (const __nv_bfloat16*)w_out, b_out, (const __nv_bfloat16*)residual));
     PIDM_LAUNCH_CHECK("linattn_block_fwd");
     return 0;
@@ -896,8 +1061,8 @@
     const int cpx = laf_chunk_px(B, N, 2);
     PIDM_CUDA(launch_plain(laf_ctx_kernel<1>, dim3(dim3((N + cpx - 1) / cpx, B)), dim3(256), LfcCfg<1>::SMEM, st, x, w, g,
                            nullptr, 0, nullptr, nullptr, dctx, N, cpx, scale, wo));
-    const int bpx = laf_chunk_px(B, N, 1);
-    PIDM_CUDA(launch_plain(laf_bwd_kernel, dim3(dim3((N + bpx - 1) / bpx, B)), dim3(256), LfbCfg::SMEM, st, x, w, g, ctx, dctx,
+    const int bpx = laf_chunk_px(B, N, 1, 64);
+    PIDM_CUDA(launch_plain(laf_bwd_kernel, dim3(dim3((N + bpx - 1) / bpx, B)), dim3(LFB_WG * 128), LAF_BWD_SMEM, st, x, w, g, ctx, dctx,
                            kmax, kzinv, (__nv_bfloat16*)dxn, N, bpx, scale, wo));
     PIDM_LAUNCH_CHECK("linattn_block_bwd");
     return 0;
diff --git a/physicsinformeddiffusionmodels_b200/csrc/hopper.cuh b/physicsinformeddiffusionmodels_b200/csrc/hopper.cuh
--- a/physicsinformeddiffusionmodels_b200/csrc/hopper.cuh
+++ b/physicsinformeddiffusionmodels_b200/csrc/hopper.cuh
@@ -108,6 +108,19 @@
         : "memory");
 }
 
+__device__ __forceinline__ void wgmma_bf16_rs(float (&d)[16], const uint32_t (&a)[4], uint64_t db, uint32_t scale_d) {
+    asm volatile(
+        "{\n\t.reg .pred p;\n\t"
+        "setp.ne.b32 p, %21, 0;\n\t"
+        "wgmma.mma_async.sync.aligned.m64n32k16.f32.bf16.bf16 "
+        "{%0, %1, %2, %3, %4, %5, %6, %7, %8, %9, %10, %11, %12, %13, %14, %15}, "
+        "{%16, %17, %18, %19}, %20, p, 1, 1, 0;\n\t}"
+        : "+f"(d[0]), "+f"(d[1]), "+f"(d[2]), "+f"(d[3]), "+f"(d[4]), "+f"(d[5]), "+f"(d[6]), "+f"(d[7]), "+f"(d[8]), "+f"(d[9]), "+f"(d[10]), "+f"(d[11]), "+f"(d[12]), "+f"(d[13]), "+f"(d[14]), "+f"(d[15])
+        : "r"(a[0]), "r"(a[1]), "r"(a[2]), "r"(a[3]), "l"(db), "r"(scale_d)
+        : "memory");
+}
+__device__ __forceinline__ void fence_proxy_async() { asm volatile("fence.proxy.async.shared::cta;" ::: "memory"); }
+
 typedef CUresult (*EncodeTiledFn)(CUtensorMap*, CUtensorMapDataType, cuuint32_t, void*, const cuuint64_t*,
                                   const cuuint64_t*, const cuuint32_t*, const cuuint32_t*, CUtensorMapInterleave,
                                   CUtensorMapSwizzle, CUtensorMapL2promotion, CUtensorMapFloatOOBfill);
```

Result: faster. 7496, median of 6 (+1.9%).
